# amathislab/BUCTD

Measured on AMD Instinct MI355X. Metric: images/sec (train) BUCTD-CoAM-W48 384x288, higher is better.
Workload: dtype f32 (3x3 convs: operands split exactly into 3 bf16 pieces, 6 bf16 MFMAs per product, fp32 accumulate - fp32-class); 1 GPU; BUCTD-CoAM-W48 (pose_hrnet_coam, ATT_MODULES [F,T,F,F], colored condition) 384x288 CrowdPose-14kpt full train step: fwd + JointsMSE + bwd + grad all-reduce + Adam + arg-max accuracy decode; global_batch=32, batch_per_gpu=32, input=N x 6 x 384 x 288 fp32, params=115581770, parallelism=dp1, hip_streams=4, conv_math=bf16x6, step_graph=False

## Files before the change

### buctd_amd/_C.py

```python
import ctypes as C
import os

import torch

_HERE = os.path.dirname(os.path.abspath(__file__))
LIB_PATH = os.path.join(_HERE, "lib", "libbuctd_hip.so")


class ConvDesc(C.Structure):
    _fields_ = [(n, C.c_int) for n in ("N", "H", "W", "Ci", "Co", "R", "S", "stride", "pad", "Ho", "Wo")]


class BasicBlockDesc(C.Structure):
    _fields_ = ([(n, C.c_int) for n in ("N", "H", "W", "C")] +
                [(n, C.c_void_p) for n in ("x", "w1_fwd", "w2_fwd", "w1_bwd", "w2_bwd", "gamma1", "beta1", "gamma2", "beta2",
                                           "running_mean1", "running_var1", "running_mean2", "running_var2")] +
                [(n, C.c_float) for n in ("eps1", "momentum1", "eps2", "momentum2")] +
                [(n, C.c_void_p) for n in ("z1", "z2", "y", "acc", "stat")])


class BasicBlockGrads(C.Structure):
    _fields_ = ([(n, C.c_void_p) for n in ("dy", "dz2", "dres", "dy1", "dz1", "dx", "dw1", "dw2", "dgamma1", "dbeta1",
                                           "dgamma2", "dbeta2")] +
                [(n, C.c_int) for n in ("acc_w1", "acc_w2", "acc_bn1", "acc_bn2")] +
                [("bn_acc", C.c_void_p), ("wg_ws", C.c_void_p), ("wg_ws_bytes", C.c_size_t)])


class BnAccIn(C.Structure):
    _fields_ = [("acc", C.c_void_p), ("rows", C.c_long), ("eps", C.c_float), ("momentum", C.c_float),
                ("mean_out", C.c_void_p), ("invstd_out", C.c_void_p), ("running_mean", C.c_void_p),
                ("running_var", C.c_void_p)]


class C3Conv(C.Structure):
    _fields_ = ([(n, C.c_int) for n in ("N", "H", "W", "Ci", "Co")] +
                [(n, C.c_void_p) for n in ("x", "wprep", "residual")] + [("relu", C.c_int)] +
                [(n, C.c_void_p) for n in ("y", "stats_acc")] + [("in_bn", C.POINTER(BnAccIn))] +
                [(n, C.c_void_p) for n in ("in_gamma", "in_beta")] + [("in_relu", C.c_int)] +
                [(n, C.c_void_p) for n in ("bn_z", "bn_y", "bn_mean", "bn_invstd", "bn_gamma", "bn_beta", "bn_acc")])


class C3ConvEval(C.Structure):
    _fields_ = ([(n, C.c_int) for n in ("N", "H", "W", "Ci", "Co")] +
                [(n, C.c_void_p) for n in ("x", "wprep", "scale", "shift", "residual")] + [("relu", C.c_int), ("y", C.c_void_p)])


class BnApplyItem(C.Structure):
    _fields_ = [("z", C.c_void_p), ("st", BnAccIn), ("gamma", C.c_void_p), ("beta", C.c_void_p), ("residual", C.c_void_p),
                ("relu", C.c_int), ("y", C.c_void_p), ("rows", C.c_long), ("C", C.c_int)]


class BnBwdItem(C.Structure):
    _fields_ = ([(n, C.c_void_p) for n in ("dy", "y", "z", "mean", "invstd", "gamma", "beta")] +
                [("relu", C.c_int), ("rows", C.c_long), ("C", C.c_int)] +
                [(n, C.c_void_p) for n in ("dz", "dres", "dgamma", "dbeta")] +
                [("accumulate", C.c_int), ("acc", C.c_void_p), ("acc_ready", C.c_int)])


class Wg3Conv(C.Structure):
    _fields_ = ([(n, C.c_int) for n in ("N", "H", "W", "Ci", "Co")] +
                [(n, C.c_void_p) for n in ("x", "dy", "dw")] + [("accumulate", C.c_int)] +
                [(n, C.c_void_p) for n in ("x_mean", "x_invstd", "x_gamma", "x_beta")] + [("x_relu", C.c_int)] +
                [("workspace", C.c_void_p), ("workspace_bytes", C.c_size_t)])


class MhaArgs(C.Structure):
    _fields_ = ([(n, C.c_int) for n in ("B", "T", "h", "dh")] +
                [(n, C.c_void_p) for n in ("q", "k", "v")] + [(n, C.c_int) for n in ("ldq", "ldk", "ldv")] +
                [("out", C.c_void_p), ("ldo", C.c_int), ("lse", C.c_void_p), ("scale", C.c_float), ("p_drop", C.c_float),
                 ("dout", C.c_void_p), ("lddo", C.c_int)] +
                [(n, C.c_void_p) for n in ("dq", "dk", "dv")] + [(n, C.c_int) for n in ("lddq", "lddk", "lddv")])


class AttnRowsArgs(C.Structure):
    _fields_ = ([(n, C.c_int) for n in ("B", "T", "h", "dh", "R")] + [("q", C.c_void_p), ("k", C.c_void_p)] +
                [("ldq", C.c_int), ("ldk", C.c_int), ("rows", C.c_void_p), ("scale", C.c_float), ("out", C.c_void_p),
                 ("out_heads", C.c_void_p)])


class RefineArgs(C.Structure):
    _fields_ = ([(n, C.c_void_p) for n in ("coords", "maxvals", "offset", "center", "scale", "box_score", "items",
                                           "cond_trunc", "cond_joints", "status", "hist_preds", "hist_score",
                                           "hist_box_score", "hist_keypoint_score", "hist_center", "hist_scale")] +
                [(n, C.c_int) for n in ("B", "K", "pass_", "passes", "heatmap_w", "heatmap_h", "crop_w", "crop_h")] +
                [(n, C.c_double) for n in ("margin", "aspect_ratio", "in_vis_thre", "scale_thre")])


class SampleGeomArgs(C.Structure):
    _fields_ = ([(n, C.c_void_p) for n in ("joints", "joints_vis", "cond", "cond_vis", "center", "scale", "bbox",
                                           "half_body", "draws", "bbox_draws", "flags", "pair", "items", "out_joints",
                                           "out_joints_vis", "out_cond", "out_cond_vis", "cond_trunc", "target_xy",
                                           "target_vis", "out_center", "out_scale", "out_rotation", "status")] +
                [(n, C.c_int) for n in ("B", "K", "crop_w", "crop_h", "keep_rect", "bbox_aug")] +
                [(n, C.c_double) for n in ("margin", "aspect_ratio", "scale_thre", "stride_x", "stride_y")])


class KptMatchArgs(C.Structure):
    _fields_ = ([(n, C.c_int) for n in ("images", "K", "n_thr", "n_area")] + [(n, C.c_long) for n in ("dt_total", "gt_total")] +
                [(n, C.c_void_p) for n in ("dt_offsets", "gt_offsets", "oks_offsets", "dt_kpts", "gt_kpts", "gt_area",
                                           "gt_bbox", "gt_flags", "sigmas", "thresholds", "area_ranges", "oks",
                                           "dt_matched", "dt_ignored")])


class VisCanvas(C.Structure):
    _fields_ = [("base", C.c_void_p), ("row_stride", C.c_long), ("H", C.c_int), ("W", C.c_int)]


class VisPoseArgs(C.Structure):
    _fields_ = ([(n, C.c_void_p) for n in ("canvases", "person_offsets", "persons", "joints", "skeleton", "palette",
                                           "tiles")] +
                [(n, C.c_int) for n in ("C", "P", "K", "L", "n_palette", "n_tiles", "canvas_h_max", "canvas_w_max",
                                        "style", "thickness", "radius")] +
                [("score_thresh", C.c_float), ("alpha256", C.c_int)])


VIS_POSE_PLAIN, VIS_POSE_PRETTY = 0, 1
VIS_POSE_TILE_W, VIS_POSE_TILE_H, VIS_POSE_CHUNK = 64, 16, 256


GRAD_SUMSQ_CHUNK = 8192

STEP_MAX_GROUPS, STEP_CHUNK = 16, 16384


class StepChunk(C.Structure):
    _fields_ = [("start", C.c_long), ("len", C.c_int), ("group", C.c_int)]


class AdamGroup(C.Structure):
    _fields_ = ([(n, C.c_float) for n in ("lr", "beta1", "beta2", "eps", "weight_decay")] +
                [("decoupled", C.c_int), ("step", C.c_int)])


class SgdGroup(C.Structure):
    _fields_ = [(n, C.c_float) for n in ("lr", "momentum", "weight_decay")] + [("nesterov", C.c_int)]


class AvgItem(C.Structure):
    _fields_ = [("src", C.c_void_p), ("avg", C.c_void_p), ("n", C.c_long)]


class MatmulDesc(C.Structure):
    _fields_ = [
        ("batch", C.c_int), ("M", C.c_int), ("N", C.c_int), ("K", C.c_int),
        ("a_layout", C.c_int), ("b_layout", C.c_int),
        ("lda", C.c_int), ("ldb", C.c_int), ("ldc", C.c_int),
        ("stride_a", C.c_long), ("stride_b", C.c_long), ("stride_c", C.c_long),
        ("Kc", C.c_int), ("group_stride_a", C.c_long), ("group_stride_bk", C.c_long),
        ("Nc", C.c_int), ("group_stride_bn", C.c_long), ("group_stride_c", C.c_long),
        ("alpha", C.c_float), ("bias_axis", C.c_int),
    ]


_P = C.c_void_p
_I = C.c_int
_L = C.c_long
_F = C.c_float
_D = C.c_double
_U64 = C.c_uint64
_SZ = C.c_size_t
_PD = C.POINTER(ConvDesc)
_PM = C.POINTER(MatmulDesc)
_PI = C.POINTER(C.c_int)
_PL = C.POINTER(C.c_long)

SIGNATURES = {
    "buctd_version": (_I, []),
    "buctd_last_error": (C.c_char_p, []),
    "buctd_conv2d_fwd": (_I, [_PD, _P, _P, _P, _P, _P, _P, _I, _P, _P, _P]),
    "buctd_conv2d_fwd_thin": (_I, [_PD]),
    "buctd_conv2d_dgrad": (_I, [_PD, _P, _P, _P, _P, _P, _P]),
    "buctd_conv2d_stats_groups": (_I, [_PD, _I, _PI, _PI]),
    "buctd_conv2d_wgrad_workspace": (_SZ, [_PD]),
    "buctd_conv2d_wgrad": (_I, [_PD, _P, _P, _P, _I, _P, _SZ, _P]),
    "buctd_conv2d_plan": (_I, [_PD, _I, _I, _PI]),
    "buctd_matmul_workspace": (_SZ, [_PM]),
    "buctd_matmul": (_I, [_PM, _P, _P, _P, _P, _P, _SZ, _P]),
    "buctd_matmul_plan": (_I, [_PM, _P, _P, _PI]),
    "buctd_bn_finalize": (_I, [_P, _P, _I, _I, _L, _I, _F, _F, _P, _P, _P, _P, _P]),
    "buctd_conv3x3_bf16x3_supported": (_I, [_I, _I, _I, _I, _I]),
    "buctd_conv3x3_bf16x3_stats_groups": (_I, [_I, _I, _I, _I, _I, _PI, _PI]),
    "buctd_conv3x3_bf16x3_prep_bytes": (_SZ, [_I, _I, _I]),
    "buctd_conv3x3_bf16x3_prep": (_I, [_I, _I, _P, _I, _P, _P]),
    "buctd_conv3x3_bf16x3_prep_batched": (_I, [_P, _I, _L, _P]),
    "buctd_conv3x3_bf16x3": (_I, [_I, _I, _I, _I, _I, _P, _P, _P, _P, _P, _P, _I, _P, _P, _P, _P]),
    "buctd_conv3x3_wgrad_bf16x3_supported": (_I, [_I, _I, _I, _I, _I]),
    "buctd_conv3x3_wgrad_bf16x3_workspace": (_SZ, [_I, _I, _I, _I, _I]),
    "buctd_conv3x3_wgrad_bf16x3": (_I, [_I, _I, _I, _I, _I, _P, _P, _P, _I, _P, _SZ, _P]),
    "buctd_conv3x3_bf16x6_supported": (_I, [_I, _I, _I, _I, _I]),
    "buctd_conv3x3_bf16x6_stats_groups": (_I, [_I, _I, _I, _I, _I, _PI, _PI]),
    "buctd_conv3x3_bf16x6_prep_bytes": (_SZ, [_I, _I, _I]),
    "buctd_conv3x3_bf16x6_prep": (_I, [_I, _I, _P, _I, _P, _P]),
    "buctd_conv3x3_bf16x6": (_I, [_I, _I, _I, _I, _I, _P, _P, _P, _P, _P, _P, _I, _P, _P, _P, _P]),
    "buctd_bn_bwd_from_partials": (_I, [_P, _P, _P, _P, _P, _P, _P, _I, _L, _I, _P, _I, _P, _P, _P, _P, _I, _P, _SZ, _P]),
    "buctd_conv3x3_wgrad_bf16x6_bnin": (_I, [_I, _I, _I, _I, _I, _P, _P, _P, _I, _P, _P, _P, _P, _I, _P, _SZ, _P]),
    "buctd_conv3x3_wgrad_bf16x6_supported": (_I, [_I, _I, _I, _I, _I]),
    "buctd_conv3x3_wgrad_bf16x6_workspace": (_SZ, [_I, _I, _I, _I, _I]),
    "buctd_conv3x3_wgrad_bf16x6": (_I, [_I, _I, _I, _I, _I, _P, _P, _P, _I, _P, _SZ, _P]),
    "buctd_bn_stats": (_I, [_P, _L, _I, _P, _PI, _PI, _P]),
    "buctd_bn_stats_groups": (_I, [_L, _I, _PI, _PI]),
    "buctd_bn_apply": (_I, [_P, _P, _P, _P, _P, _P, _I, _P, _L, _I, _P]),
    "buctd_bn_bwd_workspace": (_SZ, [_L, _I]),
    "buctd_bn_bwd": (_I, [_P, _P, _P, _P, _P, _P, _P, _I, _L, _I, _P, _P, _P, _P, _I, _P, _SZ, _P]),
    "buctd_bn_fold": (_I, [_P, _P, _P, _P, _F, _I, _P, _P, _P]),
    "buctd_bn_acc_bytes": (_SZ, [_I]),
    "buctd_bn_apply_acc": (_I, [_P, C.POINTER(BnAccIn), _P, _P, _P, _I, _P, _L, _I, _P]),
    "buctd_bn_bwd_acc": (_I, [_P, _P, _P, _P, _P, _P, _P, _I, _L, _I, _P, _P, _P, _P, _I, _P, _I, _P]),
    "buctd_conv3x3_bf16x6_acc": (_I, [_I] * 5 + [_P, _P, _P, _I, _P, _P, C.POINTER(BnAccIn), _P, _P, _I, _P]),
    "buctd_conv3x3_bf16x6_bnstat_acc": (_I, [_I] * 5 + [_P] * 12),
    "buctd_gconv_x6_fwd_acc": (_I, [_I] * 6 + [_P] * 6),
    "buctd_conv3x3_bf16x6_group": (_I, [_I, C.POINTER(C3Conv), _P]),
    "buctd_conv3x3_bf16x6_group_eval": (_I, [_I, C.POINTER(C3ConvEval), _P]),
    "buctd_conv3x3_bf16x6_group_workgroups": (_I, [_I, C.POINTER(C3Conv)]),
    "buctd_conv3x3_bf16x6_plan": (_I, [_I, _I, _I, _I, _I, _I, C.POINTER(C.c_int)]),
    "buctd_conv3x3_wgrad_bf16x6_plan": (_I, [_I, _I, _I, _I, _I, C.POINTER(C.c_int)]),
    "buctd_gconv_wgrad_x6_supported": (_I, [_I] * 6),
    "buctd_gconv_wgrad_x6_plan": (_I, [_I] * 6 + [C.POINTER(C.c_int)]),
    "buctd_gconv_wgrad_x6_workspace": (_SZ, [_I] * 6),
    "buctd_gconv_wgrad_x6": (_I, [_I] * 6 + [_P, _P, _P, _I, _P, _SZ, _P]),
    "buctd_bn_apply_acc_group": (_I, [_I, C.POINTER(BnApplyItem), _P]),
    "buctd_bn_bwd_acc_group": (_I, [_I, C.POINTER(BnBwdItem), _P]),
    "buctd_conv3x3_wgrad_bf16x6_group_workspace": (_SZ, [_I] * 6),
    "buctd_conv3x3_wgrad_bf16x6_group": (_I, [_I, C.POINTER(Wg3Conv), _P]),
    "buctd_conv3x3_wgrad_bf16x6_group_workgroups": (_I, [_I, C.POINTER(Wg3Conv)]),
    "buctd_stream_fork": (_I, [_P, _P]),
    "buctd_basic_branches_fwd_train": (_I, [_I, _I, C.POINTER(BasicBlockDesc), _P]),
    "buctd_basic_branches_bwd": (_I, [_I, _I, C.POINTER(BasicBlockDesc), C.POINTER(BasicBlockGrads), _P, _P]),
    "buctd_basic_chain_fwd_train": (_I, [_I, C.POINTER(BasicBlockDesc), _P]),
    "buctd_basic_chain_bwd": (_I, [_I, C.POINTER(BasicBlockDesc), C.POINTER(BasicBlockGrads), _P, _P]),
    "buctd_x6_image_dims": (_I, [_I, _I, _I, _P, _P]),
    "buctd_x6_image_bytes": (C.c_size_t, [_I, _I, _I]),
    "buctd_x6_image": (_I, [_P, _I, _I, _I, _L, _L, _I, _L, _L, _I, _P, _P]),
    "buctd_x6_gemm": (_I, [_I, _I, _I, _P, _P, _P, _I, _F, _P, _L, _I, _L, _P]),
    "buctd_x6_gemm_plan": (_I, [_I, _I, _I, _PI]),
    "buctd_x6_gemm_tile": (_I, [_I, _I, _I, _I, _PI, _PI]),
    "buctd_x6_image_path": (_I, [_P, _I, _I, _I, _L, _L, _I, _L, _L, _I, _I, _I, _PI]),
    "buctd_add": (_I, [_P, _P, _P, _L, _I, _P]),
    "buctd_add_n": (_I, [C.POINTER(_P), _I, _P, _L, _P]),
    "buctd_mul": (_I, [_P, _P, _P, _L, _P]),
    "buctd_scale": (_I, [_P, _P, _F, _P, _L, _P]),
    "buctd_copy_channels": (_I, [_P, _L, _I, _I, _P, _I, _I, _I, _P]),
    "buctd_add_bcast": (_I, [_P, _P, _P, _L, _L, _P]),
    "buctd_batch_sum": (_I, [_P, _L, _L, _P, _I, _P]),
    "buctd_relu_bwd": (_I, [_P, _P, _P, _L, _P]),
    "buctd_colsum_workspace": (_SZ, [_L, _I]),
    "buctd_colsum": (_I, [_P, _L, _I, _P, _I, _P, _SZ, _P]),
    "buctd_nchw_to_nhwc": (_I, [_P, _I, _I, _I, _I, _I, _I, _P, _P]),
    "buctd_nhwc_to_nchw": (_I, [_P, _I, _I, _I, _I, _P, _P]),
    "buctd_fuse_sum": (_I, [C.POINTER(_P), _PI, _I, _I, _I, _I, _I, _I, _P, _P]),
    "buctd_fuse_sum_bwd": (_I, [_P, _P, _I, _I, _I, _I, _I, _P, _P]),
    "buctd_resize_bilinear": (_I, [_P, _I, _I, _I, _I, _I, _I, _I, _I, _P, _P]),
    "buctd_maxpool3x3s2_fwd": (_I, [_P, _I, _I, _I, _I, _P, _P, _P]),
    "buctd_maxpool3x3s2_bwd": (_I, [_P, _P, _I, _I, _I, _I, _P, _P]),
    "buctd_softmax_dropout_fwd": (_I, [_P, _L, _I, _F, _F, _U64, _P, _P, _P]),
    "buctd_softmax_dropout_bwd": (_I, [_P, _P, _L, _I, _F, _F, _U64, _P, _P]),
    "buctd_softmax_dropout_fwd_dseed": (_I, [_P, _L, _I, _F, _F, _P, _P, _P, _P]),
    "buctd_softmax_dropout_bwd_dseed": (_I, [_P, _P, _L, _I, _F, _F, _P, _P, _P]),
    "buctd_dropout": (_I, [_P, _P, _L, _F, _U64, _P]),
    "buctd_dropout_dseed": (_I, [_P, _P, _L, _F, _P, _P]),
    "buctd_dropout_seed_fill": (_I, [_P, _I, _U64, _U64, _P]),
    "buctd_attn_smallqk_supported": (_I, [_I, _I, _I]),
    "buctd_attn_smallqk_plan": (_I, [_I, _I, _I, _I, _F, _I, _PI]),
    "buctd_attn_smallqk_fwd": (_I, [_I, _I, _I, _I, _P, _P, _P, _F, _F, _U64, _I, _P, _P, _P, _P]),
    "buctd_attn_smallqk_bwd": (_I, [_I, _I, _I, _I, _P, _P, _P, _P, _P, _P, _P, _F, _F, _U64, _I, _P, _P, _P, _P, _P]),
    "buctd_attn_smallqk_fwd_dseed": (_I, [_I, _I, _I, _I, _P, _P, _P, _F, _F, _P, _I, _P, _P, _P, _P]),
    "buctd_attn_smallqk_bwd_dseed": (_I, [_I, _I, _I, _I, _P, _P, _P, _P, _P, _P, _P, _F, _F, _P, _I, _P, _P, _P, _P, _P]),
    "buctd_layernorm_fwd": (_I, [_P, _P, _P, _L, _I, _F, _P, _P, _P, _P]),
    "buctd_add_layernorm_fwd": (_I, [_P, _P, _P, _P, _L, _I, _F, _P, _P, _P, _P, _P]),
    "buctd_layernorm_bwd_workspace": (_SZ, [_L, _I]),
    "buctd_layernorm_bwd": (_I, [_P, _P, _P, _P, _P, _L, _I, _P, _P, _P, _I, _P, _SZ, _P]),
    "buctd_joints_mse": (_I, [_P, _P, _P, _I, _I, _I, _P, _P, _F, _P, _SZ, _P]),
    "buctd_joints_ohkm_mse_workspace": (_SZ, [_I, _I]),
    "buctd_joints_ohkm_mse": (_I, [_P, _P, _P, _I, _I, _I, _I, _P, _P, _F, _P, _SZ, _P]),
    "buctd_argmax_decode": (_I, [_P, _I, _I, _I, _P, _P, _P, _P]),
    "buctd_warp_affine_norm": (_I, [_P, _I, _I, _I, _P, _P, _P, _L, _P, _P]),
    "buctd_cond_render_into": (_I, [_P, _I, _P, _I, _I, _I, _I, _I, _I, _P, _L, _P, _SZ, _P]),
    "buctd_cond_geometry": (_I, [_P, _P, _P, _P, _I, _I, _P, _P, _P, _P]),
    "buctd_cond_mirror": (_I, [_P, _I, _P, _P, _I, _I, _I, _P, _P]),
    "buctd_mirror_rows": (_I, [_P, _L, _P, _L, _P, _I, _I, _I, _I, _I, _P]),
    "buctd_refine_step": (_I, [C.POINTER(RefineArgs), _P]),
    "buctd_sample_geometry": (_I, [C.POINTER(SampleGeomArgs), _P]),
    "buctd_synthesize_pose": (_I, [_P, _P, _P, _P, _P, _P, _I, _I, _I, C.c_ulonglong, _P, _P]),
    "buctd_gconv_x6_supported": (_I, [_I] * 7),
    "buctd_gconv_x6_prep_bytes": (_SZ, [_I, _I, _I, _I]),
    "buctd_gconv_x6_prep": (_I, [_I, _I, _I, _P, _I, _P, _P]),
    "buctd_gconv_x6_prep_item_bytes": (_SZ, []),
    "buctd_gconv_x6_prep_item": (_I, [_I, _I, _I, _P, _I, _P, _P]),
    "buctd_gconv_x6_prep_batched": (_I, [_P, _I, _P]),
    "buctd_gconv_x6_stats_groups": (_I, [_I] * 6 + [_PI, _PI]),
    "buctd_gconv_x6_fwd": (_I, [_I] * 6 + [_P] * 6 + [_I, _P, _P, _P, _P]),
    "buctd_gconv_x6_dgrad": (_I, [_I] * 6 + [_P] * 4 + [_P]),
    "buctd_gconv_x6_plan": (_I, [_I] * 8 + [C.POINTER(C.c_int)]),
    "buctd_mha_fwd_bf16x6_workspace": (_SZ, [_I, _I, _I]),
    "buctd_mha_heads_fwd_bf16x6_ws": (_I, [C.POINTER(MhaArgs), _P, _SZ, _P]),
    "buctd_mha_heads_fwd_supported": (_I, [_I, _I, _I]),
    "buctd_mha_heads_fwd": (_I, [C.POINTER(MhaArgs), _P]),
    "buctd_mha_heads_fwd_bf16x6": (_I, [C.POINTER(MhaArgs), _P]),
    "buctd_mha_heads_train_supported": (_I, [_I, _I, _I]),
    "buctd_mha_heads_fwd_train": (_I, [C.POINTER(MhaArgs), _U64, _P]),
    "buctd_mha_heads_bwd_workspace": (_SZ, [_I, _I, _I]),
    "buctd_mha_heads_bwd": (_I, [C.POINTER(MhaArgs), _U64, _P, _SZ, _P]),
    "buctd_mha_heads_fwd_train_dseed": (_I, [C.POINTER(MhaArgs), _P, _P]),
    "buctd_mha_heads_bwd_dseed": (_I, [C.POINTER(MhaArgs), _P, _P, _SZ, _P]),
    "buctd_attn_rows_supported": (_I, [_I, _I, _I]),
    "buctd_attn_rows": (_I, [C.POINTER(AttnRowsArgs), _P]),
    "buctd_nms_workspace": (_SZ, [_I]),
    "buctd_nms": (_I, [_P, _P, _P, _I, _I, _F, _P, _SZ, _P]),
    "buctd_cpu_nms": (_I, [_P, _I, _P, _F, _P, _P]),
    "buctd_kpt_rescore": (_I, [_P, _P, _I, _I, _D, _P, _P, _P, _P]),
    "buctd_oks_nms_grouped": (_I, [_P, _I, _I, _P, _P, _P, _I, _D, _I, _D, _P, _P]),
    "buctd_coco_kpt_match_workspace": (_SZ, [_L, _I, _I]),
    "buctd_coco_kpt_match": (_I, [C.POINTER(KptMatchArgs), _P, _SZ, _P]),
    "buctd_kpt_crowding": (_I, [_P, _I, _L, _I, _P, _P, _P, _P, _D, _P, _P, _P]),
    "buctd_kpt_segment_ap": (_I, [_P, _I, _I, _L, _P, _P, _I, _I, _P, _P, _I, _I, _I, _P, _P, _P]),
    "buctd_pose_boxes": (_I, [_P, _I, _I, _I, _P, _D, _P, _P, _P]),
    "buctd_match_boxes": (_I, [_P, _P, _I, _P, _P, _P, _P, _P, _P]),
    "buctd_group_max_iou": (_I, [_P, _I, _P, _I, _P, _P, _P, _P]),
    "buctd_group_near_list": (_I, [_P, _I, _P, _P, _P, _P]),
    "buctd_vis_minmax": (_I, [_P, _I, _I, _I, _L, _L, _L, _L, _P, _P]),
    "buctd_vis_heatmap_grid": (_I, [_P, _I, _I, _I, _L, _L, _L, _L, _P, _P, _I, _I, _I, _P, _I, _P, _P]),
    "buctd_vis_joint_grid": (_I, [_P, _I, _I, _I, _L, _L, _L, _L, _P, _I, _P, _P, _P, _P, _P, _P, _I, _I, _I, _P, _P]),
    "buctd_vis_pose_overlay": (_I, [C.POINTER(VisPoseArgs), _P]),
    "buctd_argmax_decode_refined": (_I, [_P, _I, _I, _I, _P, _P, _P, _P, _P]),
    "buctd_argmax_decode_dark": (_I, [_P, _I, _I, _I, _P, _P, _P, _P, _P]),
    "buctd_gaussian_target": (_I, [_P, _P, _I, _I, _I, _I, _F, _F, _F, _P, _P, _P]),
    "buctd_cond_render_workspace": (_SZ, [_I, _I, _I, _I]),
    "buctd_cond_render": (_I, [_P, _I, _P, _I, _I, _I, _I, _I, _I, _P, _P, _SZ, _P]),
    "buctd_flipback_avg": (_I, [_P, _P, _P, _I, _I, _I, _I, _I, _P, _P]),
    "buctd_sgd_step": (_I, [_P, _P, _P, _L, _F, _F, _F, _I, _I, _F, _P]),
    "buctd_adam_step": (_I, [_P, _P, _P, _P, _L, _F, _F, _F, _F, _I, _F, _P]),
    "buctd_sgd_step_dscale": (_I, [_P, _P, _P, _L, _F, _F, _F, _I, _I, _F, _P, _P]),
    "buctd_adam_step_dscale": (_I, [_P, _P, _P, _P, _L, _F, _F, _F, _F, _I, _F, _P, _P]),
    "buctd_step_chunks": (_L, [_PL, _PI, _I, C.POINTER(StepChunk)]),
    "buctd_adam_step_groups": (_I, [_P, _P, _P, _P, _P, _L, C.POINTER(AdamGroup), _I, _F, _P, _P]),
    "buctd_sgd_step_groups": (_I, [_P, _P, _P, _P, _L, C.POINTER(SgdGroup), _I, _F, _P, _P]),
    "buctd_grad_sumsq_workspace": (_SZ, [_PL, _I]),
    "buctd_grad_sumsq": (_I, [_P, _PL, _I, _P, _P, _SZ, _P]),
    "buctd_grad_clip_coef": (_I, [_P, _D, _D, _P, _P, _P]),
    "buctd_grad_segment_stats": (_I, [_P, _P, _I, _P, _P, _P]),
    "buctd_ema_update": (_I, [_P, _P, _L, _F, _P]),
    "buctd_ema_update_tensors": (_I, [_P, _I, _F, _P]),
    "buctd_swap": (_I, [_P, _P, _L, _P]),
    "buctd_bf16_pack_conv": (_I, [_P, _L, _L, _L, _L, _I, _I, _I, _P, _P, _P, _P, _P, _F, _P, _P, _P]),
    "buctd_bf16_conv": (_I, [_P, _I, _I, _I, _I, _P, _P, _I, _I, _I, _I, _P, _I, _I, _P, _P, _SZ, _P]),
    "buctd_bf16_fuse_sum": (_I, [C.POINTER(_P), _PI, _I, _I, _I, _I, _I, _I, _P, _P]),
    "buctd_bf16_from_f32": (_I, [_P, _L, _P, _P]),
}

_lib = None


class BuctdHipError(RuntimeError):
    pass


def lib():
    global _lib
    if _lib is None:
        if not os.path.isfile(LIB_PATH):
            raise BuctdHipError(
                f"{LIB_PATH} is missing - build it with `make` (or __graft_entry__.build()); "
                "buctd_amd has no CPU / eager fallback")
        handle = C.CDLL(LIB_PATH, mode=C.RTLD_GLOBAL)
        for name, (res, args) in SIGNATURES.items():
            fn = getattr(handle, name)
            fn.restype = res
            fn.argtypes = args
        _lib = handle
    return _lib


def check(rc, what=""):
    if rc != 0:
        msg = lib().buctd_last_error()
        raise BuctdHipError(f"{what} failed ({rc}): {msg.decode() if msg else ''}")


_raw_stream = getattr(torch._C, "_cuda_getCurrentRawStream", None)
_raw_device = getattr(torch._C, "_cuda_getDevice", None)


def current_stream_handle():
# ... 16 lines not shown
```

### buctd_amd/csrc/block.hip

```cpp
#include "common.h"
#include "../../include/buctd_hip.h"
#include <string.h>

#define BLK_TRY(call)      \
  do {                     \
    const int rc_ = (call); \
    if (rc_) return rc_;   \
  } while (0)

static bool fwd_ptrs_ok(const buctd_basic_block& b) {
  return b.x && b.w1_fwd && b.w2_fwd && b.z1 && b.z2 && b.y && b.acc && b.stat;
}

static bool bwd_ptrs_ok(const buctd_basic_block& b, const buctd_basic_block_grads& g) {
  return b.x && b.w1_bwd && b.w2_bwd && b.z1 && b.z2 && b.y && b.stat && g.dy && g.dres && g.dy1 && g.dw1 && g.dw2 && g.bn_acc &&
         g.wg_ws && g.dz2 && g.dz1;
}


static float* mean1_of(const buctd_basic_block& b) { return b.stat; }
static float* invstd1_of(const buctd_basic_block& b) { return b.stat + b.C; }
static float* mean2_of(const buctd_basic_block& b) { return b.stat + 2 * b.C; }
static float* invstd2_of(const buctd_basic_block& b) { return b.stat + 3 * b.C; }
static void* acc1_of(void* acc) { return acc; }
static void* acc2_of(void* acc, int C) { return (char*)acc + buctd_bn_acc_bytes(C); }

static void acc_in_of(const buctd_basic_block& b, int second, buctd_bn_acc_in* st) {
  st->acc = second ? acc2_of(b.acc, b.C) : acc1_of(b.acc);
  st->rows = (long)b.N * b.H * b.W;
  st->eps = second ? b.eps2 : b.eps1;
  st->momentum = second ? b.momentum2 : b.momentum1;
  st->mean_out = second ? mean2_of(b) : mean1_of(b);
  st->invstd_out = second ? invstd2_of(b) : invstd1_of(b);
  st->running_mean = second ? b.running_mean2 : b.running_mean1;
  st->running_var = second ? b.running_var2 : b.running_var1;
}

static buctd_c3_conv c3_of(const buctd_basic_block& b) {
  buctd_c3_conv c;
  memset(&c, 0, sizeof(c));
  c.N = b.N; c.H = b.H; c.W = b.W; c.Ci = c.Co = b.C;
  return c;
}

static int stream_fork(hipStream_t from, hipStream_t to, const char* who) {
  if (from == to) return BUCTD_OK;
  static thread_local hipEvent_t evs[16] = {nullptr};
  int devid = 0;
  if (hipGetDevice(&devid) != hipSuccess || devid < 0 || devid >= 16) {
    buctd_set_error("%s: cannot identify the current device", who);
    return BUCTD_ELAUNCH;
  }
  hipEvent_t& ev = evs[devid];
  if (!ev && hipEventCreateWithFlags(&ev, hipEventDisableTiming) != hipSuccess) {
    buctd_set_error("%s: hipEventCreate failed", who);
    return BUCTD_ELAUNCH;
  }
  if (hipEventRecord(ev, from) != hipSuccess || hipStreamWaitEvent(to, ev, 0) != hipSuccess) {
    buctd_set_error("%s: stream fork failed", who);
    return BUCTD_ELAUNCH;
  }
  return BUCTD_OK;
}

static int issue_conv_fwd(bool group, int n, const buctd_c3_conv* c, void* s) {
  if (group) return buctd_conv3x3_bf16x6_group(n, c, s);
  return buctd_conv3x3_bf16x6_acc(c->N, c->H, c->W, c->Ci, c->Co, c->x, c->wprep, c->residual, c->relu, c->y, c->stats_acc,
                                  c->in_bn, c->in_gamma, c->in_beta, c->in_relu, s);
}
static int issue_dgrad(bool group, int n, const buctd_c3_conv* c, void* s) {
  if (group) return buctd_conv3x3_bf16x6_group(n, c, s);
  if (c->bn_acc)
    return buctd_conv3x3_bf16x6_bnstat_acc(c->N, c->H, c->W, c->Ci, c->Co, c->x, c->wprep, c->residual, c->y, c->bn_z, c->bn_y,
                                           c->bn_mean, c->bn_invstd, c->bn_gamma, c->bn_beta, c->bn_acc, s);
  return buctd_conv3x3_bf16x6(c->N, c->H, c->W, c->Ci, c->Co, c->x, c->wprep, nullptr, nullptr, nullptr, c->residual, 0, c->y,
                              nullptr, nullptr, s);
}
static int issue_wgrad(bool group, int n, const buctd_wg3_conv* c, void* s) {
  if (group) return buctd_conv3x3_wgrad_bf16x6_group(n, c, s);
  if (c->x_mean)
    return buctd_conv3x3_wgrad_bf16x6_bnin(c->N, c->H, c->W, c->Ci, c->Co, c->x, c->dy, c->dw, c->accumulate, c->x_mean,
                                           c->x_invstd, c->x_gamma, c->x_beta, c->x_relu, c->workspace, c->workspace_bytes, s);
  return buctd_conv3x3_wgrad_bf16x6(c->N, c->H, c->W, c->Ci, c->Co, c->x, c->dy, c->dw, c->accumulate, c->workspace,
                                    c->workspace_bytes, s);
}
static int issue_bn_apply(bool group, int n, const buctd_bn_apply_item* a, void* s) {
  if (group) return buctd_bn_apply_acc_group(n, a, s);
  return buctd_bn_apply_acc(a->z, &a->st, a->gamma, a->beta, a->residual, a->relu, a->y, a->rows, a->C, s);
}
static int issue_bn_bwd(bool group, int n, const buctd_bn_bwd_item* i, void* s) {
  if (group) return buctd_bn_bwd_acc_group(n, i, s);
  return buctd_bn_bwd_acc(i->dy, i->y, i->z, i->mean, i->invstd, i->gamma, i->beta, i->relu, i->rows, i->C, i->dz, i->dres,
                          i->dgamma, i->dbeta, i->accumulate, i->acc, i->acc_ready, s);
}

#define BR_MAX 4

static int row_fwd_train(bool group, int nb, int n, const buctd_basic_block* blocks, void* stream) {
  for (int k = 0; k < n; ++k) {
    buctd_c3_conv cv[BR_MAX];
    buctd_bn_acc_in st1[BR_MAX];
    buctd_bn_apply_item ap[BR_MAX];
    for (int b = 0; b < nb; ++b) {
      const buctd_basic_block& B = blocks[b * n + k];
      buctd_c3_conv& c = cv[b] = c3_of(B);
      c.x = B.x; c.wprep = B.w1_fwd; c.y = B.z1; c.stats_acc = acc1_of(B.acc);
    }
    BLK_TRY(issue_conv_fwd(group, nb, cv, stream));
    for (int b = 0; b < nb; ++b) {
      const buctd_basic_block& B = blocks[b * n + k];
      buctd_c3_conv& c = cv[b];
      acc_in_of(B, 0, &st1[b]);
      c.x = B.z1; c.wprep = B.w2_fwd; c.y = B.z2; c.stats_acc = acc2_of(B.acc, B.C);
      c.in_bn = &st1[b]; c.in_gamma = B.gamma1; c.in_beta = B.beta1; c.in_relu = 1;
    }
    BLK_TRY(issue_conv_fwd(group, nb, cv, stream));
    for (int b = 0; b < nb; ++b) {
      const buctd_basic_block& B = blocks[b * n + k];
      buctd_bn_apply_item& a = ap[b];
      a.z = B.z2;
      acc_in_of(B, 1, &a.st);
      a.gamma = B.gamma2; a.beta = B.beta2; a.residual = B.x; a.relu = 1; a.y = B.y;
      a.rows = a.st.rows; a.C = B.C;
    }
    BLK_TRY(issue_bn_apply(group, nb, ap, stream));
  }
  return BUCTD_OK;
}

static bool bn2_sums_chain(const buctd_basic_block* b, const buctd_basic_block_grads* g) {
  return g->dx && g->dx == g[-1].dy && g[-1].bn_acc && b[-1].y == b->x && b[-1].N == b->N && b[-1].H == b->H && b[-1].W == b->W &&
         b[-1].C == b->C;
}

static int row_bwd(bool group, const char* who, int nb, int n, const buctd_basic_block* blocks,
                   const buctd_basic_block_grads* grads, void* stream, void* side_stream) {
  hipStream_t main_s = (hipStream_t)stream, side_s = side_stream ? (hipStream_t)side_stream : main_s;
  bool ready[BR_MAX] = {false, false, false, false};
  for (int k = n - 1; k >= 0; --k) {
    buctd_bn_bwd_item bi[BR_MAX];
    buctd_wg3_conv wg[BR_MAX];
    buctd_c3_conv cv[BR_MAX];
    bool chain[BR_MAX];
    for (int b = 0; b < nb; ++b) {
      const buctd_basic_block& B = blocks[b * n + k];
      const buctd_basic_block_grads& G = grads[b * n + k];
      chain[b] = k > 0 && bn2_sums_chain(&B, &G);
      bi[b] = buctd_bn_bwd_item{G.dy, B.y, B.z2, mean2_of(B), invstd2_of(B), B.gamma2, nullptr, 1, (long)B.N * B.H * B.W, B.C,
                                G.dz2, G.dres, G.dgamma2, G.dbeta2, G.acc_bn2, acc2_of(G.bn_acc, B.C), ready[b] ? 1 : 0};
    }
    BLK_TRY(issue_bn_bwd(group, nb, bi, stream));
    BLK_TRY(stream_fork(main_s, side_s, who));
    for (int b = 0; b < nb; ++b) {
      const buctd_basic_block& B = blocks[b * n + k];
      const buctd_basic_block_grads& G = grads[b * n + k];
      wg[b] = buctd_wg3_conv{B.N, B.H, B.W, B.C, B.C, B.z1, G.dz2, G.dw2, G.acc_w2, mean1_of(B), invstd1_of(B), B.gamma1, B.beta1,
                             1, G.wg_ws, G.wg_ws_bytes};
    }
    BLK_TRY(issue_wgrad(group, nb, wg, side_s));
    for (int b = 0; b < nb; ++b) {
      const buctd_basic_block& B = blocks[b * n + k];
      const buctd_basic_block_grads& G = grads[b * n + k];
      buctd_c3_conv& c = cv[b] = c3_of(B);
      c.x = G.dz2; c.wprep = B.w2_bwd; c.y = G.dy1;
      c.bn_z = B.z1; c.bn_mean = mean1_of(B); c.bn_invstd = invstd1_of(B); c.bn_gamma = B.gamma1; c.bn_beta = B.beta1;
      c.bn_acc = acc1_of(G.bn_acc);
    }
    BLK_TRY(issue_dgrad(group, nb, cv, stream));
    for (int b = 0; b < nb; ++b) {
      const buctd_basic_block& B = blocks[b * n + k];
      const buctd_basic_block_grads& G = grads[b * n + k];
      bi[b] = buctd_bn_bwd_item{G.dy1, nullptr, B.z1, mean1_of(B), invstd1_of(B), B.gamma1, B.beta1, 1, (long)B.N * B.H * B.W, B.C,
                                G.dz1, nullptr, G.dgamma1, G.dbeta1, G.acc_bn1, acc1_of(G.bn_acc), 1};
    }
    BLK_TRY(issue_bn_bwd(group, nb, bi, stream));
    BLK_TRY(stream_fork(main_s, side_s, who));
    for (int b = 0; b < nb; ++b) {
      const buctd_basic_block& B = blocks[b * n + k];
      const buctd_basic_block_grads& G = grads[b * n + k];
      wg[b] = buctd_wg3_conv{B.N, B.H, B.W, B.C, B.C, B.x, G.dz1, G.dw1, G.acc_w1, nullptr, nullptr, nullptr, nullptr, 0,
                             G.wg_ws, G.wg_ws_bytes};
    }
    BLK_TRY(issue_wgrad(group, nb, wg, side_s));
    int m = 0;
    for (int b = 0; b < nb; ++b) {
      const buctd_basic_block& B = blocks[b * n + k];
      const buctd_basic_block_grads& G = grads[b * n + k];
      ready[b] = chain[b];
      if (!G.dx) continue;
      buctd_c3_conv& c = cv[m++] = c3_of(B);
      c.x = G.dz1; c.wprep = B.w1_bwd; c.residual = G.dres; c.y = G.dx;
      if (chain[b]) {
        const buctd_basic_block& Bp = blocks[b * n + k - 1];
        c.bn_z = Bp.z2; c.bn_y = Bp.y; c.bn_mean = mean2_of(Bp); c.bn_invstd = invstd2_of(Bp); c.bn_gamma = Bp.gamma2;
        c.bn_acc = acc2_of(grads[b * n + k - 1].bn_acc, B.C);
      }
    }
    if (m) BLK_TRY(issue_dgrad(group, m, cv, stream));
  }
  return BUCTD_OK;
}

extern "C" int buctd_basic_chain_fwd_train(int n, const buctd_basic_block* blocks, void* stream) {
  BUCTD_CHECK_ARG(n > 0 && blocks, "buctd_basic_chain_fwd_train: bad argument");
  for (int k = 0; k < n; ++k) BUCTD_CHECK_ARG(fwd_ptrs_ok(blocks[k]), "buctd_basic_chain_fwd_train: null pointer in block %d", k);
  return row_fwd_train(false, 1, n, blocks, stream);
}
extern "C" int buctd_basic_chain_bwd(int n, const buctd_basic_block* blocks, const buctd_basic_block_grads* grads, void* stream,
                                     void* side_stream) {
  BUCTD_CHECK_ARG(n > 0 && blocks && grads, "buctd_basic_chain_bwd: bad argument");
  for (int k = 0; k < n; ++k)
    BUCTD_CHECK_ARG(bwd_ptrs_ok(blocks[k], grads[k]), "buctd_basic_chain_bwd: null pointer in block %d", k);
  return row_bwd(false, "buctd_basic_chain_bwd", 1, n, blocks, grads, stream, side_stream);
}

extern "C" int buctd_basic_branches_fwd_train(int nb, int n, const buctd_basic_block* blocks, void* stream) {
  BUCTD_CHECK_ARG(nb > 0 && nb <= BR_MAX && n > 0 && blocks, "buctd_basic_branches_fwd_train: 1..%d branches", BR_MAX);
  for (int i = 0; i < nb * n; ++i)
    BUCTD_CHECK_ARG(fwd_ptrs_ok(blocks[i]), "buctd_basic_branches_fwd_train: null pointer in block %d", i);
  return row_fwd_train(true, nb, n, blocks, stream);
}
extern "C" int buctd_basic_branches_bwd(int nb, int n, const buctd_basic_block* blocks, const buctd_basic_block_grads* grads,
                                        void* stream, void* side_stream) {
  BUCTD_CHECK_ARG(nb > 0 && nb <= BR_MAX && n > 0 && blocks && grads, "buctd_basic_branches_bwd: 1..%d branches", BR_MAX);
  for (int i = 0; i < nb * n; ++i)
    BUCTD_CHECK_ARG(bwd_ptrs_ok(blocks[i], grads[i]), "buctd_basic_branches_bwd: null pointer in block %d", i);
  return row_bwd(true, "buctd_basic_branches_bwd", nb, n, blocks, grads, stream, side_stream);
}

extern "C" int buctd_stream_fork(void* from, void* to) {
  return stream_fork((hipStream_t)from, (hipStream_t)to, "buctd_stream_fork");
}
```

### buctd_amd/csrc/bn.hip

```cpp
#include "common.h"
#include "../../include/buctd_hip.h"
#include "bn_acc.h"

#define STAT_ROWS 64

__global__ __launch_bounds__(256) void bn_stats_kernel(const float* __restrict__ z, long rows, int C,
                                                       float* __restrict__ part) {
  const long r0 = (long)blockIdx.x * STAT_ROWS;
  long r1 = r0 + STAT_ROWS;
  if (r1 > rows) r1 = rows;
  const int cnt = (int)(r1 - r0);
  for (int c = threadIdx.x; c < C; c += 256) {
    float s = 0.f;
    for (long r = r0; r < r1; ++r) s += z[r * C + c];
    const float mean = cnt > 0 ? s / (float)cnt : 0.f;
    float m2 = 0.f;
    for (long r = r0; r < r1; ++r) {
      const float d = z[r * C + c] - mean;
      m2 += d * d;
    }
    part[((long)blockIdx.x * C + c) * 2 + 0] = mean;
    part[((long)blockIdx.x * C + c) * 2 + 1] = m2;
  }
}
// ... 760 lines not shown
      f32x4 g[4], zz[4], yy[4];
#pragma unroll
      for (int u = 0; u < 4; ++u) {
        const long o = (r + u * step) * c4n + tc;
        g[u] = reinterpret_cast<const f32x4*>(dy)[o];
        zz[u] = reinterpret_cast<const f32x4*>(z)[o];
        yy[u] = (relu && y) ? reinterpret_cast<const f32x4*>(y)[o] : zz[u];
      }
#pragma unroll
      for (int u = 0; u < 4; ++u) body(g[u], zz[u], yy[u]);
    }
    for (; r < r1; r += step) {
      const long o = r * c4n + tc;
      const f32x4 zz = reinterpret_cast<const f32x4*>(z)[o];
      body(reinterpret_cast<const f32x4*>(dy)[o], zz, (relu && y) ? reinterpret_cast<const f32x4*>(y)[o] : zz);
    }
  }
  sm[0][threadIdx.x] = s1;
  sm[1][threadIdx.x] = s2;
  __syncthreads();
  if (tr == 0) {
    for (int k = 1; k < rl; ++k) {
      s1 += sm[0][k * c4n + tc];
      s2 += sm[1][k * c4n + tc];
    }
    sm[0][tc] = s1;
    sm[1][tc] = s2;
  }
  __syncthreads();
  const unsigned shard = bnacc_shard();
  for (int c = threadIdx.x; c < C; c += 256)
    bnacc_add(acc, C, shard, c, (double)reinterpret_cast<const float*>(&sm[0][0])[c], (double)reinterpret_cast<const float*>(&sm[1][0])[c]);
}
__global__ __launch_bounds__(256) void bn_bwd_reduce_acc_kernel(BnBwdArgs p) {
  __shared__ f32x4 sm[2][256];
  bn_bwd_reduce_acc_body(p, blockIdx.x, sm);
}
__global__ __launch_bounds__(256) void bn_bwd_reduce_acc_group_kernel(BnGroup<BnBwdArgs> g_) {
  __shared__ f32x4 sm[2][256];
  const BnGroup<BnBwdArgs>& g = *(const BnGroup<BnBwdArgs>*)__builtin_amdgcn_kernarg_segment_ptr();
  unsigned bid, nblk;
  const int k = bn_group_find(g, &bid, &nblk);
  bn_bwd_reduce_acc_body(g.s[k], bid, sm);
}

__device__ __forceinline__ void bn_bwd_apply_acc_body(const BnBwdArgs& p, unsigned bid, unsigned nblk, unsigned char* lds_raw) {
  const float* __restrict__ dy = p.dy;
  const float* __restrict__ y = p.y;
  const float* __restrict__ z = p.z;
  const float* __restrict__ mean = p.mean;
  const float* __restrict__ invstd = p.invstd;
  const float* __restrict__ gamma = p.gamma;
  const float* __restrict__ beta = p.beta;
  const long long* __restrict__ acc = p.acc;
  float* __restrict__ dz = p.dz;
  float* __restrict__ dres = p.dres;
  float* __restrict__ dgamma = p.dgamma;
  float* __restrict__ dbeta = p.dbeta;
  const int relu = p.relu, C = p.C, accumulate = p.accumulate;
  const long total = p.rows * C;
  const float inv_rows = p.inv_rows;
  long long* wsum = reinterpret_cast<long long*>(lds_raw);
  float* tab = reinterpret_cast<float*>(lds_raw + (size_t)BNACC_WORDS * C * sizeof(long long));
  const long n4 = total >> 2;
  const long step = (long)nblk * 256;
  const bool ld_y = relu && y;
  long i = (long)bid * 256 + threadIdx.x;
  f32x4 g0 = (f32x4){0.f, 0.f, 0.f, 0.f}, g1 = g0, z0 = g0, z1 = g0, y0 = g0, y1 = g0;
  auto fetch = [&](long j) {
    if (j < n4) {
      g0 = reinterpret_cast<const f32x4*>(dy)[j];
      z0 = reinterpret_cast<const f32x4*>(z)[j];
      if (ld_y) y0 = reinterpret_cast<const f32x4*>(y)[j];
    }
    if (j + step < n4) {
      g1 = reinterpret_cast<const f32x4*>(dy)[j + step];
      z1 = reinterpret_cast<const f32x4*>(z)[j + step];
      if (ld_y) y1 = reinterpret_cast<const f32x4*>(y)[j + step];
    }
  };
  fetch(i);
  bnacc_gather_lds(acc, C, wsum);
  for (int c = threadIdx.x; c < C; c += 256) {
    double s1, s2;
    bnacc_read_lds(wsum, C, c, &s1, &s2);
    tab[c] = mean[c];
    tab[C + c] = invstd[c];
    tab[2 * C + c] = gamma[c];
    tab[3 * C + c] = (relu && !y) ? beta[c] : 0.f;
    tab[4 * C + c] = (float)s1;
    tab[5 * C + c] = (float)s2;
    if (bid == 0) {
      if (dbeta) dbeta[c] = accumulate ? dbeta[c] + (float)s1 : (float)s1;
      if (dgamma) dgamma[c] = accumulate ? dgamma[c] + (float)s2 : (float)s2;
    }
  }
  __syncthreads();
  const int dc = (int)((step * 4) % C);
  int c = (int)((i * 4) % C) - dc;
  auto one = [&](long j, int cc, f32x4 g, f32x4 zz, f32x4 yy) {
    const f32x4 mu = *reinterpret_cast<const f32x4*>(tab + cc);
    const f32x4 is = *reinterpret_cast<const f32x4*>(tab + C + cc);
    const f32x4 ga = *reinterpret_cast<const f32x4*>(tab + 2 * C + cc);
    if (relu) {
      if (!y) {
        const f32x4 be = *reinterpret_cast<const f32x4*>(tab + 3 * C + cc);
#pragma unroll
        for (int j4 = 0; j4 < 4; ++j4) {
          const float sc = is[j4] * ga[j4];
          yy[j4] = (zz[j4] - mu[j4]) * sc + be[j4];
        }
      }
#pragma unroll
      for (int j4 = 0; j4 < 4; ++j4)
        if (!(yy[j4] > 0.f)) g[j4] = 0.f;
    }
    const f32x4 s1 = *reinterpret_cast<const f32x4*>(tab + 4 * C + cc);
    const f32x4 s2 = *reinterpret_cast<const f32x4*>(tab + 5 * C + cc);
    f32x4 o;
#pragma unroll
    for (int j4 = 0; j4 < 4; ++j4) {
      const float zh = (zz[j4] - mu[j4]) * is[j4];
      o[j4] = ga[j4] * is[j4] * (g[j4] - s1[j4] * inv_rows - zh * s2[j4] * inv_rows);
    }
    reinterpret_cast<f32x4*>(dz)[j] = o;
    if (dres) reinterpret_cast<f32x4*>(dres)[j] = g;
  };
  for (; i < n4; i += 2 * step) {
    c += dc;
    if (c >= C) c -= C;
    one(i, c, g0, z0, y0);
    c += dc;
    if (c >= C) c -= C;
    if (i + step < n4) one(i + step, c, g1, z1, y1);
    fetch(i + 2 * step);
  }
}
__global__ __launch_bounds__(256, 6) void bn_bwd_apply_acc_kernel(BnBwdArgs p) {
  extern __shared__ __attribute__((aligned(16))) unsigned char lds_raw[];
  bn_bwd_apply_acc_body(p, blockIdx.x, gridDim.x, lds_raw);
}
__global__ __launch_bounds__(256, 6) void bn_bwd_apply_acc_group_kernel(BnGroup<BnBwdArgs> g_) {
  extern __shared__ __attribute__((aligned(16))) unsigned char lds_raw[];
  const BnGroup<BnBwdArgs>& g = *(const BnGroup<BnBwdArgs>*)__builtin_amdgcn_kernarg_segment_ptr();
  unsigned bid, nblk;
  const int k = bn_group_find(g, &bid, &nblk);
  bn_bwd_apply_acc_body(g.s[k], bid, nblk, lds_raw);
}

static int bn_bwd_acc_fill(const buctd_bn_bwd_item& it, const char* who, BnBwdArgs& a, long* nb) {
  BUCTD_CHECK_ARG(it.dy && it.z && it.mean && it.invstd && it.gamma && it.dz && it.acc && it.rows > 0 && it.C > 0 && it.C % 4 == 0 &&
                      it.C / 4 <= 256,
                  "%s: bad argument (C must be a multiple of 4, <= 1024)", who);
  BUCTD_CHECK_ARG(!it.relu || it.y || it.beta, "%s: relu backward needs the forward output, or beta to rebuild its sign", who);
  a.dy = it.dy; a.y = it.y; a.z = it.z; a.mean = it.mean; a.invstd = it.invstd; a.gamma = it.gamma; a.beta = it.beta;
  a.acc = (long long*)it.acc; a.relu = it.relu; a.rows = it.rows; a.C = it.C;
  *nb = bwd2_blocks(it.rows, &a.rows_per_block);
  a.inv_rows = 1.0f / (float)it.rows;
  a.dz = it.dz; a.dres = it.dres; a.dgamma = it.dgamma; a.dbeta = it.dbeta; a.accumulate = it.accumulate;
  return BUCTD_OK;
}

extern "C" int buctd_bn_bwd_acc(const float* dy, const float* y, const float* z, const float* mean, const float* invstd,
                                const float* gamma, const float* beta, int relu, long rows, int C, float* dz, float* dres,
                                float* dgamma, float* dbeta, int accumulate, void* acc, int acc_ready, void* stream) {
  const buctd_bn_bwd_item it{dy, y, z, mean, invstd, gamma, beta, relu, rows, C, dz, dres, dgamma, dbeta, accumulate, acc, acc_ready};
  BnBwdArgs a;
  long nb;
  const int rc = bn_bwd_acc_fill(it, "buctd_bn_bwd_acc", a, &nb);
  if (rc) return rc;
  hipStream_t st = (hipStream_t)stream;
  if (!acc_ready) {
    hipLaunchKernelGGL(bn_bwd_reduce_acc_kernel, dim3((unsigned)nb), dim3(256), 0, st, a);
    BUCTD_CHECK_LAUNCH("buctd_bn_bwd_acc(reduce)");
  }
  const long total = rows * C;
  hipLaunchKernelGGL(bn_bwd_apply_acc_kernel, dim3(acc_grid(total / 4, 6)), dim3(256), (size_t)(BNACC_WORDS * 8 + 6 * 4) * C, st, a);
  BUCTD_CHECK_LAUNCH("buctd_bn_bwd_acc(apply)");
  return BUCTD_OK;
}

extern "C" int buctd_bn_bwd_acc_group(int n, const buctd_bn_bwd_item* items, void* stream) {
  BUCTD_CHECK_ARG(n > 0 && n <= BNG_MAX && items, "buctd_bn_bwd_acc_group: 1..%d tensors", BNG_MAX);
  BnGroup<BnBwdArgs> ga, gr;
  ga.n = n; gr.n = 0;
  ga.first[0] = gr.first[0] = 0;
  size_t lds = 0;
  for (int k = 0; k < n; ++k) {
    long nb;
    const int rc = bn_bwd_acc_fill(items[k], "buctd_bn_bwd_acc_group", ga.s[k], &nb);
    if (rc) return rc;
    const long total = items[k].rows * items[k].C;
    ga.first[k + 1] = ga.first[k] + (unsigned)acc_grid(total / 4, 6);
    const size_t l = (size_t)(BNACC_WORDS * 8 + 6 * 4) * items[k].C;
    if (l > lds) lds = l;
    if (!items[k].acc_ready) {
      gr.s[gr.n] = ga.s[k];
      gr.first[gr.n + 1] = gr.first[gr.n] + (unsigned)nb;
      ++gr.n;
    }
  }
  for (int k = n; k < BNG_MAX; ++k) ga.first[k + 1] = ga.first[n];
  for (int k = gr.n; k < BNG_MAX; ++k) gr.first[k + 1] = gr.first[gr.n];
  hipStream_t st = (hipStream_t)stream;
  if (gr.n) {
    hipLaunchKernelGGL(bn_bwd_reduce_acc_group_kernel, dim3(gr.first[gr.n]), dim3(256), 0, st, gr);
    BUCTD_CHECK_LAUNCH("buctd_bn_bwd_acc_group(reduce)");
  }
  hipLaunchKernelGGL(bn_bwd_apply_acc_group_kernel, dim3(ga.first[n]), dim3(256), lds, st, ga);
  BUCTD_CHECK_LAUNCH("buctd_bn_bwd_acc_group(apply)");
  return BUCTD_OK;
}
```

### buctd_amd/csrc/c3_common.h

```cpp
#pragma once
#include "common.h"
#include <stdlib.h>
#include "../../include/buctd_hip.h"
#include "bn_acc.h"

typedef __bf16 bf16x8 __attribute__((ext_vector_type(8)));
typedef unsigned short u16x4 __attribute__((ext_vector_type(4)));

#define CK 32

template <int NP> struct Geo;
template <> struct Geo<2> {
  static constexpr int ROWB = 160;
  static constexpr int PST = 64;
  static constexpr int CPR = 8;
  static constexpr int BROW = 128;
  static constexpr int BLDS = 160;
};
template <> struct Geo<3> {
  static constexpr int ROWB = 96;
  static constexpr int PST = 32;
  static constexpr int CPR = 4;
  static constexpr int BROW = 192;
  static constexpr int BLDS = 224;
};

struct C3Args {
  const float* x;
  const unsigned char* wp;
  float* out;
  const float* bias;
  const float* scale;
  const float* shift;
  const float* res;
  float* stats;
  int* counts;
  int N, H, W, Ci, Co;
  int SW, IB, P;
  int relu, na;
  const float* in_gamma;
  const float* in_beta;
  int in_relu;
  int col_major;
  unsigned ib_mul, ib_sh, sw_mul, sw_sh;
  int omap, oH, oW, ost, oy0, ox0;
  const float* bs_z;
  const float* bs_y;
  const float* bs_mean;
  const float* bs_invstd;
  const float* bs_gamma;
  const float* bs_beta;
  long long* stats_acc;
  long long* bs_acc;
  BnAccFwd in_acc;
};

#define C3G_MAX 4
struct C3Group {
  C3Args conv[C3G_MAX];
  int nconv;
  int tiles[C3G_MAX];
  int gx[C3G_MAX];
  int gy[C3G_MAX];
  int variant[C3G_MAX];
};

#define C3_EPI_EXCH_OFF 24576
#define C3_EPI_LDS (C3_EPI_EXCH_OFF + 256 * 16)

__device__ __forceinline__ int fast_div(int n, unsigned mul, unsigned sh) {
  return (int)(__umulhi((unsigned)n, mul) >> sh);
}

typedef float c3_f32x2 __attribute__((ext_vector_type(2)));
typedef __bf16 c3_bf16x2 __attribute__((ext_vector_type(2)));
typedef unsigned c3_u32x2 __attribute__((ext_vector_type(2)));
template <int NP, int PST>
__device__ __forceinline__ void split_store_pk(unsigned char* row, int c, f32x4 v) {
  c3_f32x2 lo = {v.x, v.y}, hi = {v.z, v.w};
#pragma unroll
  for (int q = 0; q < NP; ++q) {
    const unsigned a = __builtin_bit_cast(unsigned, __builtin_convertvector(lo, c3_bf16x2));
    const unsigned b = __builtin_bit_cast(unsigned, __builtin_convertvector(hi, c3_bf16x2));
    *reinterpret_cast<c3_u32x2*>(row + q * PST + 2 * c) = (c3_u32x2){a, b};
    if (q + 1 < NP) {
      lo -= (c3_f32x2){__uint_as_float(a << 16), __uint_as_float(a & 0xffff0000u)};
      hi -= (c3_f32x2){__uint_as_float(b << 16), __uint_as_float(b & 0xffff0000u)};
    }
  }
}

template <int NP, int PST>
__device__ __forceinline__ void split_store(unsigned char* row, int c, f32x4 v) {
#pragma unroll
  for (int q = 0; q < NP; ++q) {
    u16x4 pc;
#pragma unroll
    for (int j = 0; j < 4; ++j) {
      const __bf16 h = (__bf16)v[j];
      pc[j] = __builtin_bit_cast(unsigned short, h);
      v[j] -= (float)h;
    }
    *reinterpret_cast<u16x4*>(row + q * PST + 2 * c) = pc;
  }
}

#define MAX_SW 75

static inline int c3_row_width(int W) { return W + 1; }

template <int V>
struct IC { static constexpr int value = V; };

template <int MF, int NF, int WM, int WN>
__device__ __forceinline__ void c3_epilogue(const C3Args& p, f32x4 (&acc)[MF][NF], unsigned char* smem, int bx, int by,
                                            int p0, int n0) {
  const int t = threadIdx.x, lane = t & 63, wave = t >> 6;
  const int i16 = lane & 15, g = lane >> 4;
  const int wave_m = wave % WM, wave_n = wave / WM;
  constexpr int MR = MF * 16;
  constexpr int RH = (MR + 63) / 64;
  constexpr int LD = NF * 16 + 4;
  constexpr int EP = 1;
  static_assert(MR <= 128, "c3_epilogue: at most 128 rows per wave");
  float* stg = reinterpret_cast<float*>(smem) + wave * (EP * 16 * LD);
  int* rowoff = reinterpret_cast<int*>(smem) + 4 * EP * 16 * LD + wave * 128;
  unsigned long long vmask[RH];
  int cnt = 0;
#pragma unroll
  for (int h = 0; h < RH; ++h) {
    int myoff = -1;
    const int r = lane + 64 * h;
    if (r < MR) {
      const int pp = p0 + wave_m * MR + r;
      if (pp < p.P) {
        const int n = fast_div(pp, p.ib_mul, p.ib_sh);
        const int rem = pp - n * p.IB;
        const int yy = fast_div(rem, p.sw_mul, p.sw_sh), xx = rem - yy * p.SW;
        if (n < p.N && yy >= 1 && xx >= 1 && xx <= p.W)
          myoff = p.omap ? ((n * p.oH + (yy - 1) * p.ost + p.oy0) * p.oW + (xx - 1) * p.ost + p.ox0) * p.Co
                         : ((n * p.H + yy - 1) * p.W + xx - 1) * p.Co;
      }
    }
    vmask[h] = __ballot(myoff >= 0);
    cnt += __popcll(vmask[h]);
    rowoff[r] = myoff;
  }
  auto valid = [&](int row) -> bool { return (vmask[row >> 6] >> (row & 63)) & 1ull; };
  const int grp = bx * WM + wave_m;
  if (p.stats && p.counts && by == 0 && wave_n == 0 && lane == 0) p.counts[grp] = cnt;
  const int ncol0 = n0 + wave_n * NF * 16;
  float bv[NF];
#pragma unroll
  for (int nf = 0; nf < NF; ++nf) bv[nf] = p.bias ? p.bias[ncol0 + nf * 16 + i16] : 0.f;
  double2* exch = reinterpret_cast<double2*>(smem + C3_EPI_EXCH_OFF);
  if (p.stats || p.stats_acc) {
    const float inv_cnt = cnt > 0 ? 1.f / (float)cnt : 0.f;
#pragma unroll
    for (int nf = 0; nf < NF; ++nf) {
      float s1 = 0.f;
#pragma unroll
      for (int mf = 0; mf < MF; ++mf)
#pragma unroll
        for (int rg = 0; rg < 4; ++rg) s1 += valid(mf * 16 + g * 4 + rg) ? acc[mf][nf][rg] + bv[nf] : 0.f;
      s1 += __shfl_xor(s1, 16, 64);
      s1 += __shfl_xor(s1, 32, 64);
      const float mean = s1 * inv_cnt;
      float s2 = 0.f;
#pragma unroll
      for (int mf = 0; mf < MF; ++mf)
#pragma unroll
        for (int rg = 0; rg < 4; ++rg) {
          const float d = acc[mf][nf][rg] + bv[nf] - mean;
          s2 += valid(mf * 16 + g * 4 + rg) ? d * d : 0.f;
        }
      s2 += __shfl_xor(s2, 16, 64);
      s2 += __shfl_xor(s2, 32, 64);
      if (g == 0) {
        const int n = ncol0 + nf * 16 + i16;
        if (p.stats) *reinterpret_cast<float2*>(p.stats + ((long)grp * p.Co + n) * 2) = make_float2(mean, s2);
        if (p.stats_acc) {
          const double nn = (double)cnt, m = (double)mean;
          exch[wave_m * (WN * NF * 16) + wave_n * NF * 16 + nf * 16 + i16] = make_double2(nn * m, (double)s2 + nn * m * m);
        }
      }
    }
    if (p.stats_acc) {
      __syncthreads();
      if (t < WN * NF * 16) {
        double a1 = 0.0, a2 = 0.0;
#pragma unroll
        for (int w = 0; w < WM; ++w) {
          const double2 v = exch[w * (WN * NF * 16) + t];
          a1 += v.x;
          a2 += v.y;
        }
        bnacc_add(p.stats_acc, p.Co, bnacc_shard(), n0 + t, a1, a2);
      }
    }
  }
  constexpr int Q4 = NF * 4;
  constexpr int NACC = (64 % Q4 == 0) ? 1 : 3;
  static_assert(NF <= 4 && (64 % Q4 == 0 || Q4 == 12), "c3_epilogue: unexpected column count for the bs reduction");
  f32x4 bs1[NACC], bs2[NACC];
#pragma unroll
  for (int j = 0; j < NACC; ++j) bs1[j] = bs2[j] = (f32x4){0.f, 0.f, 0.f, 0.f};
  const bool bs_on = p.bs_acc != nullptr;
  const bool bs_rebuild = bs_on && p.bs_y == nullptr;
#define C3_EPI_SYNC() __builtin_amdgcn_wave_barrier()
  constexpr int NI = EP * NF;
  constexpr int NPASS = MF / EP;
  f32x4 pre_r[2][NI], pre_z[2][NI], pre_y[2][NI];
  const bool has_res = p.res != nullptr;
  const bool has_y = bs_on && !bs_rebuild;
  C3_EPI_SYNC();
  auto issue = [&](int ps, int buf) {
#pragma unroll
    for (int k = 0; k < NI; ++k) {
      const int item = lane + 64 * k;
      const int row = item / (NF * 4), c4 = item - row * (NF * 4);
      const int off = rowoff[ps * EP * 16 + row];
      const int o = off >= 0 ? off + ncol0 + c4 * 4 : 0;
      if (has_res) pre_r[buf][k] = *reinterpret_cast<const f32x4*>(p.res + o);
      if (bs_on) pre_z[buf][k] = *reinterpret_cast<const f32x4*>(p.bs_z + o);
      if (has_y) pre_y[buf][k] = *reinterpret_cast<const f32x4*>(p.bs_y + o);
    }
  };
  if (has_res || bs_on) issue(0, 0);
#pragma unroll
  for (int ps = 0; ps < NPASS; ++ps) {
    if (ps) C3_EPI_SYNC();
    if ((has_res || bs_on) && ps + 1 < NPASS) issue(ps + 1, (ps + 1) & 1);
#pragma unroll
    for (int e = 0; e < EP; ++e)
#pragma unroll
      for (int nf = 0; nf < NF; ++nf)
#pragma unroll
        for (int rg = 0; rg < 4; ++rg)
          stg[(e * 16 + g * 4 + rg) * LD + nf * 16 + i16] = acc[ps * EP + e][nf][rg] + bv[nf];
    C3_EPI_SYNC();
#pragma unroll
    for (int k = 0; k < NI; ++k) {
      const int item = lane + 64 * k;
      const int row = item / (NF * 4), c4 = item - row * (NF * 4);
      f32x4 v = *reinterpret_cast<const f32x4*>(stg + row * LD + c4 * 4);
      const int off = rowoff[ps * EP * 16 + row];
      const int n = ncol0 + c4 * 4;
      if (off >= 0) {
        if (p.scale) {
          const f32x4 sc = *reinterpret_cast<const f32x4*>(p.scale + n);
          const f32x4 sh = *reinterpret_cast<const f32x4*>(p.shift + n);
#pragma unroll
          for (int j = 0; j < 4; ++j) v[j] = v[j] * sc[j] + sh[j];
        }
        if (has_res) {
          const f32x4 r = pre_r[ps & 1][k];
#pragma unroll
          for (int j = 0; j < 4; ++j) v[j] += r[j];
        }
        if (p.relu) {
#pragma unroll
          for (int j = 0; j < 4; ++j) v[j] = fmaxf(v[j], 0.f);
        }
        *reinterpret_cast<f32x4*>(p.out + off + n) = v;
        if (bs_on) {
          const f32x4 zz = pre_z[ps & 1][k];
          const f32x4 mu = *reinterpret_cast<const f32x4*>(p.bs_mean + n);
          const f32x4 is = *reinterpret_cast<const f32x4*>(p.bs_invstd + n);
          f32x4 yy;
          if (bs_rebuild) {
            const f32x4 sc = is * *reinterpret_cast<const f32x4*>(p.bs_gamma + n);
            yy = (zz - mu) * sc + *reinterpret_cast<const f32x4*>(p.bs_beta + n);
          } else {
            yy = pre_y[ps & 1][k];
          }
          f32x4 gm = v;
#pragma unroll
          for (int j = 0; j < 4; ++j)
            if (!(yy[j] > 0.f)) gm[j] = 0.f;
          bs1[k % NACC] += gm;
          bs2[k % NACC] += gm * (zz - mu) * is;
        }
      }
    }
  }
  if (bs_on) {
    __syncthreads();
    f32x4* red = reinterpret_cast<f32x4*>(smem) + (size_t)wave * (NACC * 64 * 2);
#pragma unroll
    for (int j = 0; j < NACC; ++j) {
      red[(j * 64 + lane) * 2 + 0] = bs1[j];
      red[(j * 64 + lane) * 2 + 1] = bs2[j];
    }
    __syncthreads();
    if (lane < Q4) {
      f32x4 a1 = (f32x4){0.f, 0.f, 0.f, 0.f}, a2 = a1;
#pragma unroll
      for (int j = 0; j < NACC; ++j) {
        const int first = ((lane - (64 * j) % Q4) % Q4 + Q4) % Q4;
        for (int l = first; l < 64; l += Q4) {
          a1 += red[(j * 64 + l) * 2 + 0];
          a2 += red[(j * 64 + l) * 2 + 1];
        }
      }
#pragma unroll
      for (int j = 0; j < 4; ++j)
        exch[wave_m * (WN * NF * 16) + wave_n * NF * 16 + lane * 4 + j] = make_double2((double)a1[j], (double)a2[j]);
    }
    __syncthreads();
    if (t < WN * NF * 16) {
      double a1 = 0.0, a2 = 0.0;
#pragma unroll
      for (int w = 0; w < WM; ++w) {
        const double2 v = exch[w * (WN * NF * 16) + t];
        a1 += v.x;
        a2 += v.y;
      }
      bnacc_add(p.bs_acc, p.Co, bnacc_shard(), n0 + t, a1, a2);
    }
  }
}


static inline void magic_u32(unsigned d, unsigned* mul, unsigned* sh) {
  if (d == 1) { *mul = 0xFFFFFFFFu; *sh = 0; return; }
  unsigned l = 0;
  while ((1ull << l) < d) ++l;
  const unsigned long long m = ((1ull << (31 + l)) + d - 1) / d;
  *mul = (unsigned)m;
  *sh = l - 1;
}
```

### buctd_amd/csrc/c3_lean.h

```cpp
#pragma once
#include "c3_common.h"

enum { C3M_IN_BN = 1, C3M_STATS = 2, C3M_RES = 4, C3M_BS_REBUILD = 8, C3M_BS_Y = 16 };

#define C3_OOB 0x80000000u
__device__ __forceinline__ __amdgpu_buffer_rsrc_t c3_rsrc(const void* ptr, unsigned bytes) {
  return __builtin_amdgcn_make_buffer_rsrc(const_cast<void*>(ptr), 0, bytes, 0x00020000);
}
__device__ __forceinline__ f32x4 c3_bload(__amdgpu_buffer_rsrc_t r, unsigned off) {
  typedef unsigned u32x4_ __attribute__((ext_vector_type(4)));
  return __builtin_bit_cast(f32x4, __builtin_amdgcn_raw_buffer_load_b128(r, off, 0, 0));
}
__device__ __forceinline__ void c3_bstore(__amdgpu_buffer_rsrc_t r, unsigned off, f32x4 v) {
  typedef unsigned u32x4_ __attribute__((ext_vector_type(4)));
  __builtin_amdgcn_raw_buffer_store_b128(__builtin_bit_cast(u32x4_, v), r, off, 0, 0);
}

static inline size_t c3l_tab_bytes(int Ci, int BN) { return (size_t)3 * Ci * 4 + (size_t)4 * BN * 4; }

template <int MF, int NF, int WM, int WN, int MODE>
__device__ __forceinline__ void c3l_epilogue(const C3Args& p, f32x4 (&acc)[MF][NF], unsigned char* smem, float* tab, int p0,
                                             int n0) {
  constexpr bool STATS = (MODE & C3M_STATS) != 0, RES = (MODE & C3M_RES) != 0;
  constexpr bool BSR = (MODE & C3M_BS_REBUILD) != 0, BSY = (MODE & C3M_BS_Y) != 0, BS = BSR || BSY;
  static_assert(!(STATS && BS), "c3l_epilogue: forward statistics and backward sums never meet in one launch");
  const int t = threadIdx.x, lane = t & 63;
  const int wave = __builtin_amdgcn_readfirstlane(t >> 6);
  const int i16 = lane & 15, g = lane >> 4;
  const int wave_m = wave % WM, wave_n = wave / WM;
  constexpr int MR = MF * 16;
  constexpr int RH = (MR + 63) / 64;
  constexpr int LD = NF * 16 + 4;
  constexpr int BN = WN * NF * 16;
  constexpr int Q4 = NF * 4;
  constexpr int NACC = (64 % Q4 == 0) ? 1 : 3;
  constexpr int NI = NF;
  static_assert(MR <= 128 && NF <= 4 && (64 % Q4 == 0 || Q4 == 12), "c3l_epilogue: unexpected tile shape");
  float* stg = reinterpret_cast<float*>(smem) + wave * (16 * LD);
  int* rowoff = reinterpret_cast<int*>(smem) + 4 * 16 * LD + wave * 128;
  double2* exch = reinterpret_cast<double2*>(smem + C3_EPI_EXCH_OFF);

  const int oH = p.omap ? p.oH : p.H, oW = p.omap ? p.oW : p.W, ost = p.omap ? p.ost : 1;
  const int oy0 = p.omap ? p.oy0 : 0, ox0 = p.omap ? p.ox0 : 0;
  const unsigned obytes = (unsigned)p.N * oH * oW * p.Co * 4u;
  const __amdgpu_buffer_rsrc_t r_out = c3_rsrc(p.out, obytes);
  int cnt = 0;
  int r0 = -1;
#pragma unroll
  for (int h = 0; h < RH; ++h) {
    unsigned myoff = C3_OOB;
    const int r = lane + 64 * h;
    const int pp = p0 + wave_m * MR + r;
    const int n = fast_div(pp, p.ib_mul, p.ib_sh);
    const int rem = pp - n * p.IB;
    const int yy = fast_div(rem, p.sw_mul, p.sw_sh), xx = rem - yy * p.SW;
    if ((r < MR) & (pp < p.P) & (n < p.N) & (yy >= 1) & (xx >= 1) & (xx <= p.W))
      myoff = (unsigned)(((n * oH + (yy - 1) * ost + oy0) * oW + (xx - 1) * ost + ox0) * p.Co) * 4u;
    if (STATS) {
      const unsigned long long vm = __ballot(myoff != C3_OOB);
      cnt += __popcll(vm);
      if (r0 < 0 && vm) r0 = 64 * h + __builtin_ctzll(vm);
    }
    if (r < MR) reinterpret_cast<unsigned*>(rowoff)[r] = myoff;
  }
  const int ncol0 = n0 + wave_n * NF * 16;
  float* piv = tab + wave * (NF * 16);
  const float* btab = tab + wave_n * NF * 16;
  if constexpr (STATS) {
    r0 = r0 < 0 ? 0 : r0;
    const int mf0 = r0 >> 4, g0 = (r0 >> 2) & 3, rg0 = r0 & 3;
    float pv[NF];
#pragma unroll
    for (int nf = 0; nf < NF; ++nf) pv[nf] = 0.f;
#pragma unroll
    for (int mf = 0; mf < MF; ++mf)
      if (mf == mf0) {
#pragma unroll
        for (int nf = 0; nf < NF; ++nf)
          pv[nf] = rg0 == 0 ? acc[mf][nf][0] : rg0 == 1 ? acc[mf][nf][1] : rg0 == 2 ? acc[mf][nf][2] : acc[mf][nf][3];
      }
    if (g == g0) {
#pragma unroll
      for (int nf = 0; nf < NF; ++nf) piv[nf * 16 + i16] = pv[nf];
    }
  }
  __builtin_amdgcn_wave_barrier();

  const float* sp[NI];
  const unsigned* rp[NI];
  int c4_k[NI];
#pragma unroll
  for (int k = 0; k < NI; ++k) {
    const int item = lane + 64 * k;
    const int row = item / Q4;
    c4_k[k] = item - row * Q4;
    sp[k] = stg + row * LD + c4_k[k] * 4;
    rp[k] = reinterpret_cast<const unsigned*>(rowoff) + row;
  }
  const unsigned colb = (unsigned)ncol0 * 4u;
  f32x4 s1[NACC], s2[NACC], pq[NACC];
#pragma unroll
  for (int j = 0; j < NACC; ++j) {
    s1[j] = s2[j] = (f32x4){0.f, 0.f, 0.f, 0.f};
    if constexpr (STATS) pq[j] = *reinterpret_cast<const f32x4*>(piv + c4_k[j] * 4);
  }
  [[maybe_unused]] __amdgpu_buffer_rsrc_t r_res, r_z, r_y;
  if constexpr (RES) r_res = c3_rsrc(p.res, obytes);
  if constexpr (BS) r_z = c3_rsrc(p.bs_z, obytes);
  if constexpr (BSY) r_y = c3_rsrc(p.bs_y, obytes);
  f32x4 pre_r[2][RES ? NI : 1], pre_z[2][BS ? NI : 1], pre_y[2][BSY ? NI : 1];
  auto issue = [&](int ps, int buf) {
#pragma unroll
    for (int k = 0; k < NI; ++k) {
      const unsigned o = rp[k][ps * 16] + colb + c4_k[k] * 16;
      if constexpr (RES) pre_r[buf][k] = c3_bload(r_res, o);
      if constexpr (BS) pre_z[buf][k] = c3_bload(r_z, o);
      if constexpr (BSY) pre_y[buf][k] = c3_bload(r_y, o);
    }
  };
  if constexpr (RES || BS) issue(0, 0);
#pragma unroll
  for (int ps = 0; ps < MF; ++ps) {
    if (ps) __builtin_amdgcn_wave_barrier();
    if constexpr (RES || BS) {
      if (ps + 1 < MF) issue(ps + 1, (ps + 1) & 1);
    }
#pragma unroll
    for (int nf = 0; nf < NF; ++nf)
#pragma unroll
      for (int rg = 0; rg < 4; ++rg) stg[(g * 4 + rg) * LD + nf * 16 + i16] = acc[ps][nf][rg];
    __builtin_amdgcn_wave_barrier();
    f32x4 v[NI];
    unsigned off[NI];
#pragma unroll
    for (int k = 0; k < NI; ++k) {
      v[k] = *reinterpret_cast<const f32x4*>(sp[k]);
      off[k] = rp[k][ps * 16];
    }
#pragma unroll
    for (int k = 0; k < NI; ++k) {
      const bool ok = off[k] != C3_OOB;
      if constexpr (RES) v[k] += pre_r[ps & 1][k];
      c3_bstore(r_out, off[k] + colb + c4_k[k] * 16, v[k]);
      if constexpr (STATS) {
        f32x4 d = v[k] - pq[k % NACC];
#pragma unroll
        for (int j = 0; j < 4; ++j) d[j] = ok ? d[j] : 0.f;
        s1[k % NACC] += d;
        f32x4 q = s2[k % NACC];
#pragma unroll
        for (int j = 0; j < 4; ++j) q[j] = __builtin_fmaf(d[j], d[j], q[j]);
        s2[k % NACC] = q;
      }
      if constexpr (BS) {
        const f32x4 zz = pre_z[ps & 1][k];
        const f32x4 mu = *reinterpret_cast<const f32x4*>(btab + c4_k[k] * 4);
        const f32x4 is = *reinterpret_cast<const f32x4*>(btab + BN + c4_k[k] * 4);
        f32x4 yy;
        if constexpr (BSR) {
          const f32x4 sc = *reinterpret_cast<const f32x4*>(btab + 2 * BN + c4_k[k] * 4);
          yy = (zz - mu) * sc + *reinterpret_cast<const f32x4*>(btab + 3 * BN + c4_k[k] * 4);
        } else {
          yy = pre_y[ps & 1][k];
        }
        f32x4 gm;
#pragma unroll
        for (int j = 0; j < 4; ++j) gm[j] = (ok && yy[j] > 0.f) ? v[k][j] : 0.f;
        s1[k % NACC] += gm;
        f32x4 tm = gm * (zz - mu) * is;
        s2[k % NACC] += tm;
      }
    }
    if constexpr (STATS || BS) {
#pragma unroll
      for (int j = 0; j < NACC; ++j) asm volatile("" : "+v"(s1[j]), "+v"(s2[j]));
    }
  }
  if constexpr (STATS || BS) {
    __syncthreads();
    f32x4* red = reinterpret_cast<f32x4*>(smem) + (size_t)wave * (NACC * 64 * 2);
#pragma unroll
    for (int j = 0; j < NACC; ++j) {
      red[(j * 64 + lane) * 2 + 0] = s1[j];
      red[(j * 64 + lane) * 2 + 1] = s2[j];
    }
    __builtin_amdgcn_wave_barrier();
    if (lane < Q4) {
      if constexpr (BS) {
        f32x4 a1 = (f32x4){0.f, 0.f, 0.f, 0.f}, a2 = a1;
#pragma unroll
        for (int j = 0; j < NACC; ++j) {
          const int first = ((lane - (64 * j) % Q4) % Q4 + Q4) % Q4;
          for (int l = first; l < 64; l += Q4) {
            a1 += red[(j * 64 + l) * 2 + 0];
            a2 += red[(j * 64 + l) * 2 + 1];
          }
        }
#pragma unroll
        for (int j = 0; j < 4; ++j)
          exch[wave_m * BN + wave_n * NF * 16 + lane * 4 + j] = make_double2((double)a1[j], (double)a2[j]);
      } else {
        double a1[4] = {0.0, 0.0, 0.0, 0.0}, a2[4] = {0.0, 0.0, 0.0, 0.0};
#pragma unroll
        for (int j = 0; j < NACC; ++j) {
          const int first = ((lane - (64 * j) % Q4) % Q4 + Q4) % Q4;
          for (int l = first; l < 64; l += Q4) {
            const f32x4 u1 = red[(j * 64 + l) * 2 + 0], u2 = red[(j * 64 + l) * 2 + 1];
#pragma unroll
            for (int e = 0; e < 4; ++e) {
              a1[e] += (double)u1[e];
              a2[e] += (double)u2[e];
            }
          }
        }
        const double nn = (double)cnt;
#pragma unroll
        for (int e = 0; e < 4; ++e) {
          const double pi = (double)piv[lane * 4 + e];
          exch[wave_m * BN + wave_n * NF * 16 + lane * 4 + e] =
              make_double2(a1[e] + nn * pi, a2[e] + 2.0 * pi * a1[e] + nn * pi * pi);
        }
      }
    }
    __syncthreads();
    if (t < BN) {
      double a1 = 0.0, a2 = 0.0;
#pragma unroll
      for (int w = 0; w < WM; ++w) {
        const double2 v = exch[w * BN + t];
        a1 += v.x;
        a2 += v.y;
      }
      bnacc_add(STATS ? p.stats_acc : p.bs_acc, p.Co, bnacc_shard(), n0 + t, a1, a2);
    }
  }
}

template <int BM, bool IN_BN>
struct C3Stager {
  static constexpr int ROWB = Geo<3>::ROWB, PST = Geo<3>::PST, CPR = Geo<3>::CPR;
  static constexpr int RPP = 256 / CPR;
  static constexpr int PA = (BM + 2 * MAX_SW + 2 + RPP - 1) / RPP;
  static constexpr int P0 = (BM + 2 * 3 + 2) / RPP < PA ? (BM + 2 * 3 + 2) / RPP : PA;
  unsigned goff[PA], lrow[PA];
  f32x4 areg[PA];
  int arows, c4, prow;
  __amdgpu_buffer_rsrc_t r_x;

  __device__ __forceinline__ void init(const C3Args& p) {
    const int t = threadIdx.x;
    arows = p.na * 32;
    c4 = (t % CPR) * 4;
    prow = t / CPR;
    r_x = c3_rsrc(p.x, (unsigned)p.N * p.H * p.W * p.Ci * 4u);
#pragma unroll
    for (int q = 0; q < PA; ++q) {
      const int row = prow + RPP * q;
      lrow[q] = (unsigned)(row < arows ? row : arows - 1) * ROWB + 2 * c4;
    }
  }
  __device__ __forceinline__ void make(const C3Args& p, int p0) {
    const int halo = p.SW + 1;
#pragma unroll
    for (int q = 0; q < PA; ++q) {
      const int row = prow + RPP * q;
      const int pp = p0 - halo + row;
      const int n = fast_div(pp, p.ib_mul, p.ib_sh);
      const int rem = pp - n * p.IB;
      const int yy = fast_div(rem, p.sw_mul, p.sw_sh);
      const int xx = rem - yy * p.SW;
      const bool real = (row < arows) & (pp >= 0) & (pp < p.P) & (n < p.N) & (yy >= 1) & (xx >= 1) & (xx <= p.W);
      goff[q] = real ? (unsigned)(((n * p.H + yy - 1) * p.W + xx - 1) * p.Ci + c4) * 4u : C3_OOB;
    }
  }
  __device__ __forceinline__ void load(int c0) {
#pragma unroll
    for (int q = 0; q < P0; ++q) areg[q] = c3_bload(r_x, goff[q] + (unsigned)c0 * 4u);
#pragma unroll
    for (int q0 = P0; q0 < PA; q0 += 2)
      if (RPP * q0 < arows) {
        areg[q0] = c3_bload(r_x, goff[q0] + (unsigned)c0 * 4u);
        if (q0 + 1 < PA) areg[q0 + 1] = c3_bload(r_x, goff[q0 + 1] + (unsigned)c0 * 4u);
      }
  }
  __device__ __forceinline__ void store_pass(const C3Args& p, unsigned char* At, int q, const f32x4& mu, const f32x4& sc,
                                             const f32x4& be) {
    f32x4 v = areg[q];
    if constexpr (IN_BN) {
      const bool real = goff[q] != C3_OOB;
#pragma unroll
      for (int j = 0; j < 4; ++j) {
        const float u = (v[j] - mu[j]) * sc[j] + be[j];
        const float w = p.in_relu ? fmaxf(u, 0.f) : u;
        v[j] = real ? w : 0.f;
      }
// ... 183 lines not shown
```

### buctd_amd/csrc/conv3x3.hip

```cpp
#include "c3_common.h"
#include <string.h>

enum { C3M_IN_BN = 1, C3M_STATS = 2, C3M_RES = 4, C3M_BS_REBUILD = 8, C3M_BS_Y = 16 };
int c3_lean_launch(const C3Group& h, int fam, int mode, unsigned grid, size_t lds, hipStream_t st);

template <int NP, int MF, int NF, int WM, int WN>
__global__ __launch_bounds__(256, 2) void conv3x3_split_kernel(C3Args p) {
  using G = Geo<NP>;
  constexpr int ROWB = G::ROWB, PST = G::PST, CPR = G::CPR, BROW = G::BROW, BLDS = G::BLDS;
  constexpr int BM = WM * MF * 16, BN = WN * NF * 16;
  constexpr int RPP = 256 / CPR;
  constexpr int PA = (BM + 2 * MAX_SW + 2 + RPP - 1) / RPP;
  constexpr int BPR = BROW / 16;
  constexpr int PB = (BN * BPR + 255) / 256;
  extern __shared__ __attribute__((aligned(16))) unsigned char smem[];
  const int na = p.na;
  const int arows = na * 32;
  unsigned char* At = smem;
  unsigned char* Bt = smem + (size_t)arows * ROWB;

  const int t = threadIdx.x, lane = t & 63, wave = t >> 6;
  const int i16 = lane & 15, g = lane >> 4;
  const int wave_m = wave % WM, wave_n = wave / WM;

  int bx, by;
  {
    const unsigned gx = gridDim.x, gy = gridDim.y, total = gx * gy;
    const unsigned lin = blockIdx.y * gx + blockIdx.x;
    const unsigned xcd = lin & 7, idx = lin >> 3, per = total >> 3, rem = total & 7;
    const unsigned L = xcd < rem ? xcd * (per + 1) + idx : rem * (per + 1) + (xcd - rem) * per + idx;
    bx = (int)(L / gy);
    by = (int)(L - (unsigned)bx * gy);
  }
  const int p0 = bx * BM, n0 = by * BN;
  const int halo = p.SW + 1;
  const int c4 = (t % CPR) * 4;
  const int prow = t / CPR;

  int goff[PA];
#pragma unroll
  for (int q = 0; q < PA; ++q) {
    const int row = prow + RPP * q;
    const int pp = p0 - halo + row;
    int o = row < arows ? -1 : -2;
    if (row < arows && pp >= 0 && pp < p.P) {
      const int n = fast_div(pp, p.ib_mul, p.ib_sh);
      const int rem = pp - n * p.IB;
      const int yy = fast_div(rem, p.sw_mul, p.sw_sh);
      const int xx = rem - yy * p.SW;
      if (n < p.N && yy >= 1 && xx >= 1 && xx <= p.W) o = ((n * p.H + yy - 1) * p.W + xx - 1) * p.Ci;
    }
    goff[q] = o;
  }

  f32x4 areg[PA], breg[PB];
  auto load_a = [&](int c0, int cw) {
#pragma unroll
    for (int q = 0; q < PA; ++q)
      if (RPP * q < arows) {
        const bool ok = goff[q] >= 0 && c4 < cw * 16;
        areg[q] = *reinterpret_cast<const f32x4*>(p.x + (ok ? goff[q] + c0 + c4 : 0));
      }
  };
  auto store_a = [&](int cw) {
#pragma unroll
    for (int q = 0; q < PA; ++q)
      if (RPP * q < arows && goff[q] != -2) {
        const int row = prow + RPP * q;
        const bool ok = goff[q] >= 0 && c4 < cw * 16;
        split_store<NP, PST>(At + (size_t)row * ROWB, c4, ok ? areg[q] : (f32x4){0.f, 0.f, 0.f, 0.f});
      }
  };
  int bsrc[PB], bdst[PB];
#pragma unroll
  for (int q = 0; q < PB; ++q) {
    const int id = t + 256 * q;
    const int nl = id / BPR, pc = id - nl * BPR;
    const bool ok = nl < BN;
    bsrc[q] = ok ? (n0 + nl) * BROW + pc * 16 : 0;
    bdst[q] = ok ? nl * BLDS + pc * 16 : (nl & 15) * BLDS + BROW + (t & 1) * 16;
  }
  const long step_bytes = (long)p.Co * BROW;
  auto load_b = [&](int gs) {
    const unsigned char* src = p.wp + gs * step_bytes;
#pragma unroll
    for (int q = 0; q < PB; ++q) breg[q] = *reinterpret_cast<const f32x4*>(src + bsrc[q]);
  };
  auto store_b = [&](int buf) {
    unsigned char* dst = Bt + (size_t)buf * BN * BLDS;
#pragma unroll
    for (int q = 0; q < PB; ++q) *reinterpret_cast<f32x4*>(dst + bdst[q]) = breg[q];
  };

  f32x4 acc[MF][NF];
#pragma unroll
  for (int mf = 0; mf < MF; ++mf)
#pragma unroll
    for (int nf = 0; nf < NF; ++nf) acc[mf][nf] = (f32x4){0.f, 0.f, 0.f, 0.f};

  const int nfull = NP == 2 ? p.Ci / CK : 0;
  const int ntail = NP == 2 ? ((p.Ci % CK) ? 1 : 0) : p.Ci / 16;
  const int nchunks = nfull + ntail, last_step = nfull * 9 + ntail * 5 - 1;
  const unsigned char* abase = At + (size_t)(wave_m * MF * 16 + i16) * ROWB + (g & 1) * 16;
  const unsigned char* bbase = Bt + (size_t)(wave_n * NF * 16 + i16) * BLDS + g * 16;
  const bool lowk = g < 2;
  int gs = 0, buf = 0;

  auto run_chunk = [&](auto cw_tag) {
    constexpr int CW = decltype(cw_tag)::value;
    constexpr int NS = CW == 2 ? 9 : 5;
#pragma unroll
    for (int s = 0; s < NS; ++s) {
      load_b(gs < last_step ? gs + 1 : last_step);
      const int tap0 = CW == 2 ? s : 2 * s;
      const int tap1 = CW == 2 ? s : (2 * s + 1 < 9 ? 2 * s + 1 : 2 * s);
      const int o0 = ((tap0 / 3) * p.SW + tap0 % 3) * ROWB;
      const int o1 = ((tap1 / 3) * p.SW + tap1 % 3) * ROWB + (CW == 2 ? 32 : 0);
      const unsigned char* ap = abase + (lowk ? o0 : o1);
      const unsigned char* bp = bbase + (size_t)buf * BN * BLDS;
      bf16x8 a[NP][MF], b[NP][NF];
#pragma unroll
      for (int nf = 0; nf < NF; ++nf)
#pragma unroll
        for (int q = 0; q < NP; ++q) b[q][nf] = *reinterpret_cast<const bf16x8*>(bp + nf * 16 * BLDS + q * 64);
#pragma unroll
      for (int mf = 0; mf < MF; ++mf)
#pragma unroll
        for (int q = 0; q < NP; ++q) a[q][mf] = *reinterpret_cast<const bf16x8*>(ap + mf * 16 * ROWB + q * PST);
#pragma unroll
      for (int mf = 0; mf < MF; ++mf) {
#define C3_MMA(qa, qb)                                                                                          \
  _Pragma("unroll") for (int nf = 0; nf < NF; ++nf) acc[mf][nf] =                                                \
      __builtin_amdgcn_mfma_f32_16x16x32_bf16(a[qa][mf], b[qb][nf], acc[mf][nf], 0, 0, 0);
        if constexpr (NP == 3) {
          C3_MMA(2, 0) C3_MMA(0, 2) C3_MMA(1, 1) C3_MMA(1, 0) C3_MMA(0, 1) C3_MMA(0, 0)
        } else {
          C3_MMA(1, 0) C3_MMA(0, 1) C3_MMA(0, 0)
        }
#undef C3_MMA
      }
      store_b(buf ^ 1);
      __syncthreads();
      buf ^= 1;
      ++gs;
    }
  };

  const int cw0 = nfull > 0 ? 2 : 1;
  load_a(0, cw0);
  load_b(0);
  store_a(cw0);
  store_b(0);
  if (nchunks > 1) load_a(cw0 * 16, nfull > 1 ? 2 : 1);
  __syncthreads();
  int c_next = cw0 * 16;
  for (int ch = 0; ch < nchunks; ++ch) {
// ... 322 lines not shown
  }
  split_store<2, 64>(reinterpret_cast<unsigned char*>(it.wprep) + rown * 128, c4, v);
}

__device__ __forceinline__ void prep3_piece(const float* __restrict__ w, unsigned char* __restrict__ out, int Kc, int Nc,
                                            int flip, long idx) {
  const int k4 = (int)(idx & 7);
  const long rown = idx >> 3;
  const int n = (int)(rown % Nc), step = (int)(rown / Nc);
  const int chunk = step / 5, s = step - chunk * 5;
  const int tap = 2 * s + (k4 >> 2);
  const int cc = chunk * 16 + (k4 & 3) * 4;
  f32x4 v = (f32x4){0.f, 0.f, 0.f, 0.f};
  if (tap < 9) {
    if (!flip) v = *reinterpret_cast<const f32x4*>(w + ((long)n * 9 + tap) * Kc + cc);
    else {
#pragma unroll
      for (int j = 0; j < 4; ++j) v[j] = w[((long)(cc + j) * 9 + (8 - tap)) * Nc + n];
    }
  }
  const int lane = (k4 >> 1) * 16 + (n & 15);
  unsigned char* dst = out + (((size_t)step * (Nc / 16) + (n >> 4)) * 3) * 1024 + lane * 16;
  split_store<3, 1024>(dst, (k4 & 1) * 4, v);
}
__global__ __launch_bounds__(256) void conv3x3_prep3_kernel(const float* __restrict__ w, unsigned char* __restrict__ out,
                                                            int Kc, int Nc, int flip, long items) {
  const long idx = (long)blockIdx.x * 256 + threadIdx.x;
  if (idx >= items) return;
  prep3_piece(w, out, Kc, Nc, flip, idx);
}

struct C3Plan { int MF, NF, WM, WN, BM, BN, na; size_t lds; bool single; };


static int c3_steps(int Kc, int np) { return np == 3 ? (Kc / 16) * 5 : (Kc / CK) * 9 + ((Kc % CK) ? 5 : 0); }

static bool c3_plan(int np, int N, int H, int W, int Ci, int Co, C3Plan* pl) {
  if (N <= 0 || H <= 0 || W <= 0 || Ci <= 0 || Co <= 0 || Ci % 16 != 0 || Co % 16 != 0 || c3_row_width(W) > MAX_SW) return false;
  const int rowb = np == 3 ? Geo<3>::ROWB : Geo<2>::ROWB, blds = np == 3 ? Geo<3>::BLDS : Geo<2>::BLDS;
  const long P = (long)N * (H + 1) * c3_row_width(W) + c3_row_width(W);
  int nf, wn;
  if (Co % 96 == 0) { nf = 3; wn = 2; }
  else if (Co % 48 == 0) { nf = 3; wn = 1; }
  else if (Co % 128 == 0) { nf = 4; wn = 2; }
  else if (Co % 64 == 0) { nf = 4; wn = 1; }
  else if (Co % 32 == 0) { nf = 2; wn = 1; }
  else { nf = 1; wn = 1; }
  if (np == 2 && Co % 96 == 0 && ((P + 127) / 128) * (Co / 96) < 320) { nf = 3; wn = 1; }
  bool small = false;
  if (np == 3 && Co % 32 == 0 && ((P + 127) / 128) * ((Co + 95) / 96) < 200) { nf = 2; wn = 1; small = true; }
  int wm = 4 / wn, bn = wn * nf * 16;
  int mf = 1;
  const int cand[2] = {4, 2};
  for (int i = (nf == 4 ? 1 : 0); i < 2; ++i) {
    const long blocks = ((P + wm * cand[i] * 16 - 1) / (wm * cand[i] * 16)) * (Co / bn);
    const long need = np == 3 ? (small ? 160 : 224) : 320;
    if (blocks >= need) { mf = cand[i]; break; }
  }
  bool single = false;
  if (np == 3 && nf == 3 && wn == 1 && Co == bn) {
    const long b8 = (P + 511) / 512;
    if (b8 > 256 && b8 <= 512) {
      mf = 8; single = true;
      if ((P + 447) / 448 <= 512) mf = 7;
    }
  }
  pl->MF = mf; pl->NF = nf; pl->WM = wm; pl->WN = wn; pl->BM = wm * mf * 16; pl->BN = bn; pl->single = single;
  pl->na = (pl->BM + 2 * c3_row_width(W) + 3 + 31) / 32;
  size_t stage = (size_t)4 * (mf >= 2 ? 2 : 1) * 16 * (nf * 16 + 4) * 4 + 4 * 128 * 4;
  if (np == 3 && stage < (size_t)C3_EPI_LDS) stage = C3_EPI_LDS;
  if (np == 3) {
    const int nb = single ? 1 : 2;
    while ((size_t)nb * pl->na * 32 * rowb < stage) ++pl->na;
    pl->lds = (size_t)nb * pl->na * 32 * rowb + (size_t)3 * Ci * sizeof(float);
  } else {
    while ((size_t)pl->na * 32 * rowb < stage) ++pl->na;
    pl->lds = (size_t)pl->na * 32 * rowb + (size_t)2 * pl->BN * blds;
  }
  return pl->lds <= 160 * 1024;
}

static bool c3_np_ok(int np) { return np == 2 || np == 3; }

template <int NP, int MF, int NF, int WM, int WN>
static int c3_launch(const C3Args& a, const C3Plan& pl, hipStream_t st) {
  static unsigned char attr_done[3][BUCTD_MAX_DEVICES] = {{0}};
  void (*fn)(C3Args);
  int variant = 0;
  if constexpr (NP == 3) {
    if (MF >= 7) fn = conv3x3_x6_kernel<MF, NF, WM, WN, false, false, 2>;
    else { fn = conv3x3_x6_kernel<MF, NF, WM, WN, true, true, 2>; variant = 2; }
  }
  else fn = conv3x3_split_kernel<NP, (MF > 4 ? 4 : MF), NF, WM, WN>;
  if (const int rc = buctd_raise_lds_limit(reinterpret_cast<const void*>(fn), 160 * 1024, attr_done[variant], "conv3x3 (split bf16)"))
    return rc;
  dim3 grid(ceil_div(a.P, pl.BM), a.Co / pl.BN);
  hipLaunchKernelGGL(fn, grid, dim3(256), pl.lds, st, a);
  BUCTD_CHECK_LAUNCH("buctd_conv3x3 (split bf16)");
  return BUCTD_OK;
}

template <int NP>
static int c3_dispatch(const C3Args& a, const C3Plan& pl, hipStream_t st, bool dry = false) {
#define C3_CASE(mf, nf, wm, wn) \
  if (pl.MF == mf && pl.NF == nf && pl.WN == wn) return dry ? BUCTD_OK : c3_launch<NP, mf, nf, wm, wn>(a, pl, st);
#define C3_MF(nf, wm, wn) C3_CASE(4, nf, wm, wn) C3_CASE(2, nf, wm, wn) C3_CASE(1, nf, wm, wn)
  if constexpr (NP == 3) { C3_CASE(8, 3, 4, 1) C3_CASE(7, 3, 4, 1) C3_CASE(8, 3, 2, 2) }
  C3_MF(1, 4, 1) C3_MF(2, 4, 1) C3_MF(3, 4, 1) C3_MF(3, 2, 2)
  C3_CASE(2, 4, 4, 1) C3_CASE(1, 4, 4, 1) C3_CASE(2, 4, 2, 2) C3_CASE(1, 4, 2, 2)
#undef C3_MF
#undef C3_CASE
  buctd_set_error("conv3x3 (split bf16): no kernel for MF=%d NF=%d WN=%d", pl.MF, pl.NF, pl.WN);
  return BUCTD_EINVAL;
}

static int c3_supported(int np, int N, int H, int W, int Ci, int Co) {
  C3Plan pl;
  return c3_np_ok(np) && c3_plan(np, N, H, W, Ci, Co, &pl) ? 1 : 0;
}

static int c3_stats_groups(int np, int N, int H, int W, int Ci, int Co, int* ngroups, int* rows_per_group) {
  C3Plan pl;
  BUCTD_CHECK_ARG(ngroups && rows_per_group && c3_np_ok(np) && c3_plan(np, N, H, W, Ci, Co, &pl),
                  "buctd_conv3x3_*_stats_groups: unsupported shape");
  const long P = (long)N * (H + 1) * c3_row_width(W) + c3_row_width(W);
  *ngroups = ceil_div(P, pl.BM) * pl.WM;
  *rows_per_group = pl.MF * 16;
  return BUCTD_OK;
}

static size_t c3_prep_bytes(int np, int Ci, int Co, int flip) {
  if (!c3_np_ok(np) || Ci <= 0 || Co <= 0 || Ci % 16 != 0 || Co % 16 != 0) return 0;
  const int Kc = flip ? Co : Ci, Nc = flip ? Ci : Co;
  return (size_t)c3_steps(Kc, np) * Nc * (np == 3 ? Geo<3>::BROW : Geo<2>::BROW);
}

static int c3_prep(int np, int Ci, int Co, const float* w, int flip, void* wprep, void* stream) {
  BUCTD_CHECK_ARG(w && wprep && c3_np_ok(np), "buctd_conv3x3_*_prep: null pointer");
  BUCTD_CHECK_ARG(Ci > 0 && Co > 0 && Ci % 16 == 0 && Co % 16 == 0, "buctd_conv3x3_*_prep: Ci=%d Co=%d must be multiples of 16",
                  Ci, Co);
  const int Kc = flip ? Co : Ci, Nc = flip ? Ci : Co;
  const long pieces = (long)c3_steps(Kc, np) * Nc * 8;
  if (np == 3)
    hipLaunchKernelGGL(conv3x3_prep3_kernel, dim3(ceil_div(pieces, 256)), dim3(256), 0, (hipStream_t)stream, w,
                       (unsigned char*)wprep, Kc, Nc, flip ? 1 : 0, pieces);
  else
    hipLaunchKernelGGL(conv3x3_prep_kernel, dim3(ceil_div(pieces, 256)), dim3(256), 0, (hipStream_t)stream, w,
                       (unsigned char*)wprep, Kc, Nc, flip ? 1 : 0, pieces);
  BUCTD_CHECK_LAUNCH("buctd_conv3x3_*_prep");
  return BUCTD_OK;
}

struct C3InBn { const float* gamma; const float* beta; int relu; };
struct C3BwdStat { const float* z; const float* y; const float* mean; const float* invstd; const float* gamma; const float* beta; long long* acc; };
struct C3Acc { long long* stats_acc; const buctd_bn_acc_in* in; };

static int c3_fill_shape(int np, int N, int H, int W, int Ci, int Co, C3Args& a, C3Plan& pl) {
  BUCTD_CHECK_ARG(c3_np_ok(np) && c3_plan(np, N, H, W, Ci, Co, &pl),
                  "buctd_conv3x3 (split bf16): unsupported shape N%d H%d W%d Ci%d Co%d", N, H, W, Ci, Co);
  a.N = N; a.H = H; a.W = W; a.Ci = Ci; a.Co = Co;
  a.SW = c3_row_width(W); a.IB = (H + 1) * a.SW;
  const long P = (long)N * a.IB + a.SW;
  BUCTD_CHECK_ARG(P < 2147483647L && (long)N * H * W * (Ci > Co ? Ci : Co) < 2147483647L,
                  "buctd_conv3x3 (split bf16): tensor too large");
  a.P = (int)P;
  a.na = pl.na;
  a.omap = 0; a.oH = H; a.oW = W; a.ost = 1; a.oy0 = a.ox0 = 0;
  a.col_major = (np == 3 && Co / pl.BN >= 2 && (size_t)c3_steps(Ci, 3) * Co * Geo<3>::BROW > ((size_t)3 << 20)) ? 1 : 0;
  magic_u32((unsigned)a.IB, &a.ib_mul, &a.ib_sh);
  magic_u32((unsigned)a.SW, &a.sw_mul, &a.sw_sh);
  return BUCTD_OK;
}

static int c3_fill(int np, int N, int H, int W, int Ci, int Co, const float* x, const void* wprep, const float* bias,
                   const float* scale, const float* shift, const float* residual, int relu, float* y,
                   float* stats_partials, int* stats_counts, const C3InBn* in_bn, const C3BwdStat* bst, const C3Acc* accs,
                   C3Args& a, C3Plan& pl) {
  BUCTD_CHECK_ARG(x && wprep && y, "buctd_conv3x3 (split bf16): null tensor pointer");
  if (const int rc = c3_fill_shape(np, N, H, W, Ci, Co, a, pl)) return rc;
  BUCTD_CHECK_ARG((scale == nullptr) == (shift == nullptr), "buctd_conv3x3 (split bf16): scale and shift go together");
  BUCTD_CHECK_ARG((stats_partials == nullptr) == (stats_counts == nullptr),
                  "buctd_conv3x3 (split bf16): stats partials and counts go together");
  a.x = x; a.wp = (const unsigned char*)wprep; a.out = y; a.bias = bias; a.scale = scale; a.shift = shift;
  a.res = residual; a.stats = stats_partials; a.counts = stats_counts;
  a.relu = relu;
  a.in_gamma = a.in_beta = nullptr;
  a.in_relu = 0;
  a.stats_acc = nullptr; a.bs_acc = nullptr;
  memset(&a.in_acc, 0, sizeof(a.in_acc));
  if (accs) {
    BUCTD_CHECK_ARG(np == 3, "buctd_conv3x3: statistics accumulators need the bf16x6 kernel");
    a.stats_acc = accs->stats_acc;
    if (accs->in && accs->in->acc) {
      const buctd_bn_acc_in& i = *accs->in;
      BUCTD_CHECK_ARG(in_bn && in_bn->gamma && in_bn->beta && i.rows > 0 && i.mean_out && i.invstd_out &&
                          (i.running_mean == nullptr) == (i.running_var == nullptr),
                      "buctd_conv3x3: input BatchNorm from an accumulator needs gamma, beta, rows, mean_out and invstd_out");
      a.in_gamma = in_bn->gamma; a.in_beta = in_bn->beta; a.in_relu = in_bn->relu;
      a.in_acc.acc = (const long long*)i.acc; a.in_acc.rows = (double)i.rows; a.in_acc.eps = i.eps; a.in_acc.momentum = i.momentum;
      a.in_acc.mean_out = i.mean_out; a.in_acc.invstd_out = i.invstd_out; a.in_acc.rmean = i.running_mean; a.in_acc.rvar = i.running_var;
    }
  }
  a.bs_z = a.bs_y = a.bs_mean = a.bs_invstd = a.bs_gamma = a.bs_beta = nullptr;
  if (bst && bst->acc) {
    BUCTD_CHECK_ARG(np == 3 && bst->z && bst->mean && bst->invstd && (bst->y || (bst->gamma && bst->beta)),
                    "buctd_conv3x3: the BatchNorm-backward by-product needs the bf16x6 kernel, z, mean, invstd and y or gamma + beta");
    a.bs_z = bst->z; a.bs_y = bst->y; a.bs_mean = bst->mean; a.bs_invstd = bst->invstd; a.bs_gamma = bst->gamma;
    a.bs_beta = bst->beta; a.bs_acc = bst->acc;
  }
  return BUCTD_OK;
}

static int c3_lean_mask(int m) {
  switch (m) {
    case C3M_STATS: case C3M_STATS | C3M_IN_BN: case C3M_BS_REBUILD: case C3M_RES | C3M_BS_Y: case C3M_RES: return m;
    default: return -1;
  }
}

static int c3_lean_mode(const C3Args& a) {
  if ((long)a.N * a.H * a.W * (a.Ci > a.Co ? a.Ci : a.Co) * 4 >= 2147483648L) return -1;
  if (a.bias || a.scale || a.shift || a.relu || a.stats || a.counts || a.omap) return -1;
  if (a.in_acc.acc && (!a.in_gamma || !a.in_beta)) return -1;
  int m = 0;
  if (a.in_acc.acc) m |= C3M_IN_BN;
  if (a.stats_acc) m |= C3M_STATS;
  if (a.res) m |= C3M_RES;
  if (a.bs_acc) m |= a.bs_y ? C3M_BS_Y : C3M_BS_REBUILD;
  return c3_lean_mask(m);
}

static int c3_group_variant(const C3Plan& pl, int* fam, bool general = false) {
  struct V { int mf, nf, wm, wn; };
  static const V f0[] = {{7, 3, 4, 1}, {4, 3, 2, 2}, {2, 2, 4, 1}, {4, 3, 4, 1}, {4, 2, 4, 1}};
  static const V f1[] = {{4, 2, 4, 1}, {1, 4, 4, 1}, {2, 2, 4, 1}, {1, 2, 4, 1}, {2, 4, 4, 1}, {2, 4, 2, 2}, {1, 3, 4, 1}, {2, 3, 4, 1}};
  for (int f = 0; f < 2; ++f) {
    if (*fam >= 0 && *fam != f) continue;
    const V* l = f ? f1 : f0;
    const int n = f ? (general ? 8 : 6) : 5;
    for (int i = 0; i < n; ++i)
      if (l[i].mf == pl.MF && l[i].nf == pl.NF && l[i].wm == pl.WM && l[i].wn == pl.WN) {
        *fam = f;
        return i;
      }
  }
  return -1;
}

struct C3Dry { int kernel, fam, variant, wgs; };

static int c3_group_launch(int n, const C3Args* a, const C3Plan* pl, hipStream_t stream, bool* done, C3Dry* dry = nullptr) {
  *done = false;
  int order[C3G_MAX];
  double cost[C3G_MAX];
  int lean = c3_lean_mode(a[0]);
  for (int k = 0; k < n; ++k) {
    cost[k] = (double)pl[k].BM * pl[k].BN * a[k].Ci;
    order[k] = k;
    if (c3_lean_mode(a[k]) != lean) lean = -1;
  }
  if (n == 1 && lean < 0) return BUCTD_OK;
  int fam = -1;
  bool ok = false;
  int var[C3G_MAX];
  for (int f = 0; f < 2 && !ok; ++f) {
    ok = true;
    for (int k = 0; k < n && ok; ++k) {
      fam = f;
      var[k] = c3_group_variant(pl[k], &fam, lean < 0);
      ok = var[k] >= 0;
    }
  }
  if (!ok) return BUCTD_OK;
  for (int i = 1; i < n; ++i)
    for (int j = i; j > 0 && cost[order[j]] > cost[order[j - 1]]; --j) { const int t = order[j]; order[j] = order[j - 1]; order[j - 1] = t; }
  C3Group h;
  h.nconv = n;
  size_t lds = 0;
  unsigned per_xcd = 0;
  for (int i = 0; i < n; ++i) {
    const int k = order[i];
    h.conv[i] = a[k];
    h.gx[i] = ceil_div(h.conv[i].P, pl[k].BM);
    h.gy[i] = h.conv[i].Co / pl[k].BN;
    h.tiles[i] = h.gx[i] * h.gy[i];
    h.variant[i] = var[k];
    const size_t l = pl[k].lds + (lean >= 0 ? (size_t)4 * pl[k].BN * sizeof(float) : 0);
    if (l > lds) lds = l;
    per_xcd += ((unsigned)h.tiles[i] + 7) >> 3;
  }
  for (int i = n; i < C3G_MAX; ++i) h.tiles[i] = h.gx[i] = h.gy[i] = h.variant[i] = 0;
  if (lds > 160 * 1024) return BUCTD_OK;
  *done = true;
  if (dry) { *dry = C3Dry{1, fam, h.variant[0], (int)(per_xcd * 8)}; return BUCTD_OK; }
  if (lean >= 0) return c3_lean_launch(h, fam, lean, per_xcd * 8, lds, stream);
  static unsigned char attr_done[2][BUCTD_MAX_DEVICES] = {{0}};
  void (*fn)(C3Group) = fam ? conv3x3_x6_group_kernel<1> : conv3x3_x6_group_kernel<0>;
  if (const int rc = buctd_raise_lds_limit(reinterpret_cast<const void*>(fn), 160 * 1024, attr_done[fam], "buctd_conv3x3_bf16x6_group"))
    return rc;
  hipLaunchKernelGGL(fn, dim3(per_xcd * 8), dim3(256), lds, stream, h);
  BUCTD_CHECK_LAUNCH("buctd_conv3x3_bf16x6_group");
  return BUCTD_OK;
}

static int c3_launch_one(const C3Args& a, const C3Plan& pl, hipStream_t stream, C3Dry* dry = nullptr) {
  bool done = false;
  const int rc = c3_group_launch(1, &a, &pl, stream, &done, dry);
  if (rc || done) return rc;
  if (dry) *dry = C3Dry{0, -1, -1, ceil_div(a.P, pl.BM) * (a.Co / pl.BN)};
  return c3_dispatch<3>(a, pl, stream, dry != nullptr);
}

static int c3_run(int np, int N, int H, int W, int Ci, int Co, const float* x, const void* wprep, const float* bias,
                  const float* scale, const float* shift, const float* residual, int relu, float* y,
                  float* stats_partials, int* stats_counts, void* stream, const C3InBn* in_bn = nullptr,
                  const C3BwdStat* bst = nullptr, const C3Acc* accs = nullptr) {
  C3Args a;
  C3Plan pl;
  const int rc = c3_fill(np, N, H, W, Ci, Co, x, wprep, bias, scale, shift, residual, relu, y, stats_partials, stats_counts,
                         in_bn, bst, accs, a, pl);
  if (rc) return rc;
  return np == 3 ? c3_launch_one(a, pl, (hipStream_t)stream) : c3_dispatch<2>(a, pl, (hipStream_t)stream);
}

extern "C" int buctd_conv3x3_bf16x3_supported(int N, int H, int W, int Ci, int Co) { return c3_supported(2, N, H, W, Ci, Co); }
extern "C" int buctd_conv3x3_bf16x3_stats_groups(int N, int H, int W, int Ci, int Co, int* ngroups, int* rows_per_group) {
  return c3_stats_groups(2, N, H, W, Ci, Co, ngroups, rows_per_group);
}
extern "C" size_t buctd_conv3x3_bf16x3_prep_bytes(int Ci, int Co, int flip) { return c3_prep_bytes(2, Ci, Co, flip); }
extern "C" int buctd_conv3x3_bf16x3_prep(int Ci, int Co, const float* w, int flip, void* wprep, void* stream) {
  return c3_prep(2, Ci, Co, w, flip, wprep, stream);
}
extern "C" int buctd_conv3x3_bf16x3_prep_batched(const buctd_c3_prep_item* items_device, int n, long total_pieces,
                                                 void* stream) {
  BUCTD_CHECK_ARG(items_device && n > 0 && total_pieces > 0, "buctd_conv3x3_bf16x3_prep_batched: bad argument");
  hipLaunchKernelGGL(conv3x3_prep_batched_kernel, dim3(ceil_div(total_pieces, 256)), dim3(256), 0, (hipStream_t)stream,
                     items_device, n, total_pieces);
  BUCTD_CHECK_LAUNCH("buctd_conv3x3_bf16x3_prep_batched");
  return BUCTD_OK;
}
extern "C" int buctd_conv3x3_bf16x3(int N, int H, int W, int Ci, int Co, const float* x, const void* wprep,
                                    const float* bias, const float* scale, const float* shift, const float* residual,
                                    int relu, float* y, float* stats_partials, int* stats_counts, void* stream) {
  return c3_run(2, N, H, W, Ci, Co, x, wprep, bias, scale, shift, residual, relu, y, stats_partials, stats_counts, stream);
}

extern "C" int buctd_conv3x3_bf16x6_supported(int N, int H, int W, int Ci, int Co) { return c3_supported(3, N, H, W, Ci, Co); }
extern "C" int buctd_conv3x3_bf16x6_stats_groups(int N, int H, int W, int Ci, int Co, int* ngroups, int* rows_per_group) {
  return c3_stats_groups(3, N, H, W, Ci, Co, ngroups, rows_per_group);
}
extern "C" size_t buctd_conv3x3_bf16x6_prep_bytes(int Ci, int Co, int flip) { return c3_prep_bytes(3, Ci, Co, flip); }
extern "C" int buctd_conv3x3_bf16x6_prep(int Ci, int Co, const float* w, int flip, void* wprep, void* stream) {
  return c3_prep(3, Ci, Co, w, flip, wprep, stream);
}
extern "C" int buctd_conv3x3_bf16x6(int N, int H, int W, int Ci, int Co, const float* x, const void* wprep,
                                    const float* bias, const float* scale, const float* shift, const float* residual,
                                    int relu, float* y, float* stats_partials, int* stats_counts, void* stream) {
  return c3_run(3, N, H, W, Ci, Co, x, wprep, bias, scale, shift, residual, relu, y, stats_partials, stats_counts, stream);
}

extern "C" int buctd_conv3x3_bf16x6_acc(int N, int H, int W, int Ci, int Co, const float* x, const void* wprep,
                                        const float* residual, int relu, float* y, void* stats_acc,
                                        const buctd_bn_acc_in* in_bn, const float* in_gamma, const float* in_beta, int in_relu,
                                        void* stream) {
  C3InBn b{in_gamma, in_beta, in_relu};
  C3Acc a{(long long*)stats_acc, in_bn};
  BUCTD_CHECK_ARG(!in_bn || in_bn->acc, "buctd_conv3x3_bf16x6_acc: in_bn without an accumulator");
  return c3_run(3, N, H, W, Ci, Co, x, wprep, nullptr, nullptr, nullptr, residual, relu, y, nullptr, nullptr, stream,
                in_bn ? &b : nullptr, nullptr, &a);
}
extern "C" int buctd_conv3x3_bf16x6_bnstat_acc(int N, int H, int W, int Ci, int Co, const float* x, const void* wprep,
                                               const float* residual, float* y, const float* bn_z, const float* bn_y,
                                               const float* bn_mean, const float* bn_invstd, const float* bn_gamma,
                                               const float* bn_beta, void* bn_acc, void* stream) {
  C3BwdStat b{bn_z, bn_y, bn_mean, bn_invstd, bn_gamma, bn_beta, (long long*)bn_acc};
  BUCTD_CHECK_ARG(bn_acc, "buctd_conv3x3_bf16x6_bnstat_acc: null accumulator");
  return c3_run(3, N, H, W, Ci, Co, x, wprep, nullptr, nullptr, nullptr, residual, 0, y, nullptr, nullptr, stream, nullptr,
                &b);
}

static int c3_group_fill(int n, const buctd_c3_conv* convs, C3Args* a, C3Plan* pl) {
  for (int k = 0; k < n; ++k) {
    const buctd_c3_conv& c = convs[k];
    C3InBn ib{c.in_gamma, c.in_beta, c.in_relu};
    C3BwdStat bs{c.bn_z, c.bn_y, c.bn_mean, c.bn_invstd, c.bn_gamma, c.bn_beta, (long long*)c.bn_acc};
    C3Acc ac{(long long*)c.stats_acc, c.in_bn};
    BUCTD_CHECK_ARG(!c.in_bn || c.in_bn->acc, "buctd_conv3x3_bf16x6_group: in_bn without an accumulator");
    const int rc = c3_fill(3, c.N, c.H, c.W, c.Ci, c.Co, c.x, c.wprep, nullptr, nullptr, nullptr, c.residual, c.relu, c.y,
                           nullptr, nullptr, c.in_bn ? &ib : nullptr, c.bn_acc ? &bs : nullptr, &ac, a[k], pl[k]);
    if (rc) return rc;
  }
  return BUCTD_OK;
}

extern "C" int buctd_conv3x3_bf16x6_group(int n, const buctd_c3_conv* convs, void* stream) {
  BUCTD_CHECK_ARG(n > 0 && n <= C3G_MAX && convs, "buctd_conv3x3_bf16x6_group: 1..%d convolutions", C3G_MAX);
  C3Args a[C3G_MAX];
  C3Plan pl[C3G_MAX];
  if (const int rc0 = c3_group_fill(n, convs, a, pl)) return rc0;
  bool done = false;
  const int rc = c3_group_launch(n, a, pl, (hipStream_t)stream, &done);
  if (rc || done) return rc;
  for (int k = 0; k < n; ++k)
    if (const int rc1 = c3_launch_one(a[k], pl[k], (hipStream_t)stream)) return rc1;
  return BUCTD_OK;
}

extern "C" int buctd_conv3x3_bf16x6_group_eval(int n, const buctd_c3_conv_eval* convs, void* stream) {
  BUCTD_CHECK_ARG(n > 0 && n <= C3G_MAX && convs, "buctd_conv3x3_bf16x6_group_eval: 1..%d convolutions", C3G_MAX);
  C3Args a[C3G_MAX];
  C3Plan pl[C3G_MAX];
  for (int k = 0; k < n; ++k) {
    const buctd_c3_conv_eval& c = convs[k];
    const int rc = c3_fill(3, c.N, c.H, c.W, c.Ci, c.Co, c.x, c.wprep, nullptr, c.scale, c.shift, c.residual, c.relu, c.y,
                           nullptr, nullptr, nullptr, nullptr, nullptr, a[k], pl[k]);
    if (rc) return rc;
  }
  bool done = false;
  const int rc = n > 1 ? c3_group_launch(n, a, pl, (hipStream_t)stream, &done) : BUCTD_OK;
  if (rc || done) return rc;
  for (int k = 0; k < n; ++k)
    if (const int rc1 = c3_dispatch<3>(a[k], pl[k], (hipStream_t)stream)) return rc1;
  return BUCTD_OK;
}

extern "C" int buctd_conv3x3_bf16x6_group_workgroups(int n, const buctd_c3_conv* convs) {
  BUCTD_CHECK_ARG(n > 0 && n <= C3G_MAX && convs, "buctd_conv3x3_bf16x6_group_workgroups: 1..%d convolutions", C3G_MAX);
  C3Args a[C3G_MAX];
  C3Plan pl[C3G_MAX];
  if (const int rc0 = c3_group_fill(n, convs, a, pl)) return rc0;
  bool done = false;
  C3Dry dry{};
  const int rc = c3_group_launch(n, a, pl, nullptr, &done, &dry);
  if (rc) return rc;
  return done ? dry.wgs : 0;
}

extern "C" int buctd_conv3x3_bf16x6_plan(int N, int H, int W, int Ci, int Co, int option_set, int* out) {
  BUCTD_CHECK_ARG(out && (option_set == -1 || c3_lean_mask(option_set) >= 0),
                  "buctd_conv3x3_bf16x6_plan: option set %d is not one of the train-mode sets (or -1)", option_set);
  static const float some = 0.f;
  const float* on = &some;
  C3Args a{};
  C3Plan pl;
  if (const int rc = c3_fill_shape(3, N, H, W, Ci, Co, a, pl)) return rc;
  if (option_set >= 0) {
    if (option_set & C3M_IN_BN) { a.in_acc.acc = (const long long*)on; a.in_gamma = a.in_beta = on; }
    if (option_set & C3M_STATS) a.stats_acc = (long long*)on;
    if (option_set & C3M_RES) a.res = on;
    if (option_set & (C3M_BS_REBUILD | C3M_BS_Y)) a.bs_acc = (long long*)on;
    if (option_set & C3M_BS_Y) a.bs_y = on;
  }
  C3Dry dry{};
  if (const int rc = c3_launch_one(a, pl, nullptr, &dry)) return rc;
  const int v[11] = {pl.MF, pl.NF, pl.WM, pl.WN, pl.single ? 1 : 0, a.col_major, dry.kernel, dry.fam, dry.variant, pl.BM, pl.BN};
  for (int i = 0; i < 11; ++i) out[i] = v[i];
  return BUCTD_OK;
}
```

### buctd_amd/csrc/conv3x3_lean.hip

```cpp
#include "c3_lean.h"

template <int FAM, int MODE>
__global__ __launch_bounds__(256, 2) void conv3x3_x6_lean_kernel(C3Group g_) {
  extern __shared__ __attribute__((aligned(16))) unsigned char smem[];
  const C3Group& g = *(const C3Group*)__builtin_amdgcn_kernarg_segment_ptr();
  const unsigned lin = blockIdx.x, xcd = lin & 7;
  unsigned idx = lin >> 3;
  int c = -1;
  unsigned L = 0;
  for (int k = 0; k < g.nconv; ++k) {
    const unsigned total = (unsigned)g.tiles[k], per = total >> 3, rem = total & 7;
    const unsigned mine = per + (xcd < rem ? 1u : 0u);
    if (idx < mine) {
      L = xcd < rem ? xcd * (per + 1) + idx : rem * (per + 1) + (xcd - rem) * per + idx;
      c = k;
      break;
    }
    idx -= mine;
  }
  if (c < 0) return;
  const C3Args& p = g.conv[c];
  int bx, by;
  if (p.col_major) {
    by = (int)(L / (unsigned)g.gx[c]);
    bx = (int)(L - (unsigned)by * g.gx[c]);
  } else {
    bx = (int)(L / (unsigned)g.gy[c]);
    by = (int)(L - (unsigned)bx * g.gy[c]);
  }
  const int v = g.variant[c];
  if constexpr (FAM == 0) {
    switch (v) {
      case 0: c3l_tile<7, 3, 4, 1, false, false, MODE>(p, smem, bx, by); break;
      case 1: c3l_tile<4, 3, 2, 2, true, true, MODE>(p, smem, bx, by); break;
      case 2: c3l_tile<2, 2, 4, 1, true, true, MODE>(p, smem, bx, by); break;
      case 3: c3l_tile<4, 3, 4, 1, true, true, MODE>(p, smem, bx, by); break;
      default: c3l_tile<4, 2, 4, 1, true, true, MODE>(p, smem, bx, by); break;
    }
  } else {
    switch (v) {
      case 0: c3l_tile<4, 2, 4, 1, true, true, MODE>(p, smem, bx, by); break;
      case 1: c3l_tile<1, 4, 4, 1, true, true, MODE>(p, smem, bx, by); break;
      case 2: c3l_tile<2, 2, 4, 1, true, true, MODE>(p, smem, bx, by); break;
      case 3: c3l_tile<1, 2, 4, 1, true, true, MODE>(p, smem, bx, by); break;
      case 4: c3l_tile<2, 4, 4, 1, true, true, MODE>(p, smem, bx, by); break;
      default: c3l_tile<2, 4, 2, 2, true, true, MODE>(p, smem, bx, by); break;
    }
  }
}

int c3_lean_launch(const C3Group& h, int fam, int mode, unsigned grid, size_t lds, hipStream_t st) {
  static unsigned char attr_done[2][5][BUCTD_MAX_DEVICES] = {{{0}}};
  void (*fn)(C3Group) = nullptr;
  int mi = -1;
#define C3L_PICK(i, m)                                                                               \
  if (mode == (m)) {                                                                                 \
    mi = i;                                                                                          \
    fn = fam ? conv3x3_x6_lean_kernel<1, (m)> : conv3x3_x6_lean_kernel<0, (m)>;                      \
  }
  C3L_PICK(0, C3M_STATS)
  C3L_PICK(1, C3M_STATS | C3M_IN_BN)
  C3L_PICK(2, C3M_BS_REBUILD)
  C3L_PICK(3, C3M_RES | C3M_BS_Y)
  C3L_PICK(4, C3M_RES)
#undef C3L_PICK
  if (!fn) {
    buctd_set_error("conv3x3 (bf16x6, train mode): no kernel for option set %d", mode);
    return BUCTD_EINVAL;
  }
  if (const int rc = buctd_raise_lds_limit(reinterpret_cast<const void*>(fn), 160 * 1024, attr_done[fam ? 1 : 0][mi],
                                           "conv3x3 (bf16x6, train mode)"))
    return rc;
  hipLaunchKernelGGL(fn, dim3(grid), dim3(256), lds, st, h);
  BUCTD_CHECK_LAUNCH("conv3x3 (bf16x6, train mode)");
  return BUCTD_OK;
}
```

### buctd_amd/csrc/conv_gather_x6.hip

```cpp
#include "c3_lean.h"
#include <string.h>

#define GC_MAXT 9
#define GC_TAB_OFF (56 * 1024)

struct GcClass {
  int ntaps, nhs, nsteps;
  int oy0, ox0;
  long wp_off;
  unsigned pdy, pdx;
};

struct GcArgs {
  C3Args e;
  const float* src;
  const unsigned char* wp;
  int SH, SWd, SC, ss, cpt;
  int ncls;
  GcClass cls[4];
};

template <int MF, int NF, int WM, int WN, int MODE>
__global__ __launch_bounds__(256, 2) void gconv_x6_kernel(GcArgs p) {
  constexpr int BM = WM * MF * 16, BN = WN * NF * 16, ROWB = 96, PST = 32, BROW = 192;
// ... 443 lines not shown
              const float d = v - piv[nf];
              s1[nf] += d;
              s2[nf] = __builtin_fmaf(d, d, s2[nf]);
            }
          }
        }
        __builtin_amdgcn_wave_barrier();
#pragma unroll
        for (int k = 0; k < 4; ++k) {
          const int item = lane + 64 * k, row = item >> 4, c4 = item & 15;
          const long grow = (long)blk * 32 + mf * 16 + row;
          f32x4 v = *reinterpret_cast<const f32x4*>(stg + row * R1_LD + c4 * 4);
          if (grow < p.rows) {
            const long o = grow * Co + cg * 64 + c4 * 4;
            if (p.res) v += *reinterpret_cast<const f32x4*>(p.res + o);
            *reinterpret_cast<f32x4*>(p.out + o) = v;
          }
        }
        __builtin_amdgcn_wave_barrier();
      }
    }
  }
  if (p.stats_acc) {
    __syncthreads();
    double2* exch = reinterpret_cast<double2*>(smem);
#pragma unroll
    for (int nf = 0; nf < NFT; ++nf) {
      const double pi = (double)piv[nf], nn = (double)nrows;
      double a1 = (double)s1[nf] + nn * pi, a2 = (double)s2[nf] + 2.0 * pi * (double)s1[nf] + nn * pi * pi;
      a1 += __shfl_xor(a1, 16, 64); a1 += __shfl_xor(a1, 32, 64);
      a2 += __shfl_xor(a2, 16, 64); a2 += __shfl_xor(a2, 32, 64);
      if (g == 0) exch[wave * Co + nf * 16 + i16] = make_double2(a1, a2);
    }
    __syncthreads();
    for (int c = t; c < Co; c += 512) {
      double a1 = 0.0, a2 = 0.0;
#pragma unroll
      for (int w = 0; w < 8; ++w) {
        const double2 v = exch[w * Co + c];
        a1 += v.x;
        a2 += v.y;
      }
      bnacc_add(p.stats_acc, Co, bnacc_shard(), c, a1, a2);
    }
  }
}

static bool r1_ok(int kind, long rows, int cin, int cout) {
  if (kind != 1 || cin % 32 || (cout != 64 && cout != 128 && cout != 256)) return false;
  const size_t lds = (size_t)(cin / 32) * cout * R1_WROW + (size_t)8 * R1_STG;
  return lds <= 150 * 1024 && (size_t)8 * cout * 16 <= (size_t)(cin / 32) * cout * R1_WROW && rows >= 65536;
}

static int r1_run(long rows, int cin, int cout, int nft, const float* x, const void* wprep, const float* bias, const float* residual,
                  float* out, long long* stats_acc, hipStream_t st, const char* who) {
  R1Args a;
  a.x = x; a.wp = (const unsigned char*)wprep; a.bias = bias; a.res = residual; a.out = out; a.stats_acc = stats_acc;
  a.rows = rows; a.Ci = cin; a.Co = cout; a.nblocks = (int)((rows + 31) / 32);
  const size_t lds = (size_t)(cin / 32) * cout * R1_WROW + (size_t)8 * R1_STG;
  static unsigned char done[3][BUCTD_MAX_DEVICES] = {{0}};
  void (*fn)(R1Args) = nft == 4 ? conv1x1_rows_x6_kernel<4> : nft == 8 ? conv1x1_rows_x6_kernel<8> : conv1x1_rows_x6_kernel<16>;
  if (const int rc = buctd_raise_lds_limit(reinterpret_cast<const void*>(fn), 160 * 1024, done[nft == 4 ? 0 : nft == 8 ? 1 : 2], who))
    return rc;
  int grid = 256;
  if (grid * 8 > a.nblocks) grid = (a.nblocks + 7) / 8;
  hipLaunchKernelGGL(fn, dim3(grid), dim3(512), lds, st, a);
  BUCTD_CHECK_LAUNCH(who);
  return BUCTD_OK;
}

enum { GCF_BIAS = 1, GCF_SCALE = 2, GCF_RELU = 4, GCF_PARTIALS = 8, GCF_ACC = 16, GCF_RES = 32, GCF_ALL = 63 };

struct GcRoute {
  int route;
  int Hg, Wg, SH, SWd, SC, nout;
  long rows;
  int P;
  GcPlan pl;
  int mode;
  int ncls;
  GcClass cls[4];
  int tiles, ncol;
  int nft, ksteps;
};

static int gc_route(int kind, int dir, int N, int H, int W, int Ci, int Co, int flags, const char* who, GcRoute* r) {
  memset(r, 0, sizeof(GcRoute));
  BUCTD_CHECK_ARG(gc_geo(kind, dir, N, H, W, Ci, Co, &r->Hg, &r->Wg, &r->SH, &r->SWd, &r->SC, &r->nout),
                  "%s: unsupported shape kind %d N%d H%d W%d Ci%d Co%d", who, kind, N, H, W, Ci, Co);
  BUCTD_CHECK_ARG(!(dir && (flags & (GCF_PARTIALS | GCF_ACC))), "%s: no statistics on the data gradient", who);
  const bool bias = flags & GCF_BIAS, scale = flags & GCF_SCALE, relu = flags & GCF_RELU, partials = flags & GCF_PARTIALS,
             acc = flags & GCF_ACC, res = flags & GCF_RES;
  const int SC = r->SC, nout = r->nout;
  r->rows = (long)N * H * W;
  if (!scale && !relu && !partials && r1_ok(kind, r->rows, SC, nout)) {
    r->route = 1;
    r->nft = nout / 16;
    r->ksteps = SC / 32;
    return BUCTD_OK;
  }
  const long P = (long)N * (r->Hg + 1) * (r->Wg + 2) + r->Wg + 2;
  r->P = (int)P;
  gc_plan(nout, P, &r->pl);
  const bool par = kind == 2 && dir;
  const int cpt = SC / 16;
  r->ncls = gc_ncls(kind, dir);
  long off = 0;
  int tr[GC_MAXT], ts[GC_MAXT];
  for (int c = 0; c < r->ncls; ++c) {
    GcClass& k = r->cls[c];
    int tdy[GC_MAXT], tdx[GC_MAXT];
    k.ntaps = gc_taps(kind, dir, c, tr, ts, tdy, tdx);
    for (int t = 0; t < k.ntaps; ++t) {
      k.pdy |= (unsigned)(tdy[t] + 1) << (2 * t);
      k.pdx |= (unsigned)(tdx[t] + 1) << (2 * t);
    }
    k.nhs = k.ntaps * cpt;
    k.nsteps = (k.nhs + 1) / 2;
    k.oy0 = par ? (c >> 1) : 0; k.ox0 = par ? (c & 1) : 0;
    k.wp_off = off;
    off += (long)gc_class_bytes(k.ntaps, SC, nout);
  }
  r->tiles = (int)((P + r->pl.BM - 1) / r->pl.BM);
  r->ncol = nout / r->pl.BN;
  r->mode = -1;
  if (!bias && !scale && !relu && !partials && !(acc && res) && (long)N * H * W * (Ci > Co ? Ci : Co) * 4 < 2147483648L)
    r->mode = acc ? C3M_STATS : res ? C3M_RES : 0;
  return BUCTD_OK;
}

static int gc_run(int kind, int dir, int N, int H, int W, int Ci, int Co, const float* src, const void* wprep, const float* bias,
                  const float* scale, const float* shift, const float* residual, int relu, float* out, float* stats_partials,
                  int* stats_counts, void* stream, const char* who, long long* stats_acc = nullptr) {
  BUCTD_CHECK_ARG(src && wprep && out, "%s: null tensor pointer", who);
  BUCTD_CHECK_ARG((scale == nullptr) == (shift == nullptr), "%s: scale and shift go together", who);
  BUCTD_CHECK_ARG((stats_partials == nullptr) == (stats_counts == nullptr), "%s: stats partials and counts go together", who);
  const int flags = (bias ? GCF_BIAS : 0) | (scale ? GCF_SCALE : 0) | (relu ? GCF_RELU : 0) | (stats_partials ? GCF_PARTIALS : 0) |
                    (stats_acc ? GCF_ACC : 0) | (residual ? GCF_RES : 0);
  GcRoute r;
  if (const int rc = gc_route(kind, dir, N, H, W, Ci, Co, flags, who, &r)) return rc;
  if (r.route == 1)
    return r1_run(r.rows, r.SC, r.nout, r.nft, src, wprep, bias, residual, out, stats_acc, (hipStream_t)stream, who);
  const GcPlan& pl = r.pl;
  GcArgs a;
  C3Args& e = a.e;
  e.x = nullptr; e.wp = nullptr; e.out = out; e.bias = bias; e.scale = scale; e.shift = shift; e.res = residual;
  e.stats = stats_partials; e.counts = stats_counts;
  e.N = N; e.H = r.Hg; e.W = r.Wg; e.Ci = r.SC; e.Co = r.nout;
  e.SW = r.Wg + 2; e.IB = (r.Hg + 1) * (r.Wg + 2);
  e.P = r.P;
  e.relu = relu; e.na = 0;
  e.in_gamma = e.in_beta = nullptr; e.in_relu = 0; e.col_major = 0;
  e.bs_z = e.bs_y = e.bs_mean = e.bs_invstd = e.bs_gamma = e.bs_beta = nullptr;
  e.stats_acc = stats_acc; e.bs_acc = nullptr;
  memset(&e.in_acc, 0, sizeof(e.in_acc));
  magic_u32((unsigned)e.IB, &e.ib_mul, &e.ib_sh);
  magic_u32((unsigned)e.SW, &e.sw_mul, &e.sw_sh);
  const bool par = kind == 2 && dir;
  e.omap = par ? 1 : 0; e.oH = H; e.oW = W; e.ost = par ? 2 : 1; e.oy0 = e.ox0 = 0;
  a.src = src; a.wp = (const unsigned char*)wprep;
  a.SH = r.SH; a.SWd = r.SWd; a.SC = r.SC; a.ss = (kind == 2 && !dir) ? 2 : 1; a.cpt = r.SC / 16;
  a.ncls = r.ncls;
  for (int c = 0; c < 4; ++c) a.cls[c] = r.cls[c];
  hipStream_t st = (hipStream_t)stream;
  if (pl.NF == 3 && pl.WM == 2) gc_launch<4, 3, 2, 2>(a, r.tiles, r.ncol, st, r.mode);
  else if (pl.NF == 4 && pl.WM == 2) gc_launch<4, 4, 2, 2>(a, r.tiles, r.ncol, st, r.mode);
  else if (pl.NF == 4) gc_launch<2, 4, 4, 1>(a, r.tiles, r.ncol, st, r.mode);
  else gc_launch<2, 3, 4, 1>(a, r.tiles, r.ncol, st, r.mode);
  BUCTD_CHECK_LAUNCH(who);
  return BUCTD_OK;
}

extern "C" int buctd_gconv_x6_plan(int kind, int dir, int N, int H, int W, int Ci, int Co, int flags, int* out) {
  BUCTD_CHECK_ARG(out && (dir == 0 || dir == 1) && flags >= 0 && flags <= GCF_ALL, "buctd_gconv_x6_plan: bad argument");
  BUCTD_CHECK_ARG(!(dir && (flags & ~GCF_RES)), "buctd_gconv_x6_plan: a data gradient carries the residual only (flags %d)", flags);
  BUCTD_CHECK_ARG(!((flags & GCF_ACC) && (flags & ~(GCF_ACC | GCF_BIAS))),
                  "buctd_gconv_x6_plan: the accumulator form carries the bias only (flags %d)", flags);
  GcRoute r;
  if (const int rc = gc_route(kind, dir, N, H, W, Ci, Co, flags, "buctd_gconv_x6_plan", &r)) return rc;
  int i = 0;
  out[i++] = r.route;
  out[i++] = r.pl.MF; out[i++] = r.pl.NF; out[i++] = r.pl.WM; out[i++] = r.pl.WN; out[i++] = r.pl.BM; out[i++] = r.pl.BN;
  out[i++] = r.route ? 0 : r.mode;
  out[i++] = r.ncls;
  for (int c = 0; c < 4; ++c) { out[i++] = r.cls[c].ntaps; out[i++] = r.cls[c].nhs; out[i++] = r.cls[c].nsteps; }
  out[i++] = r.tiles; out[i++] = r.ncol;
  out[i++] = r.nft; out[i++] = r.ksteps;
  return BUCTD_OK;
}

extern "C" int buctd_gconv_x6_fwd(int kind, int N, int H, int W, int Ci, int Co, const float* x, const void* wprep,
                                  const float* bias, const float* scale, const float* shift, const float* residual, int relu,
                                  float* y, float* stats_partials, int* stats_counts, void* stream) {
  return gc_run(kind, 0, N, H, W, Ci, Co, x, wprep, bias, scale, shift, residual, relu, y, stats_partials, stats_counts, stream,
                "buctd_gconv_x6_fwd");
}

extern "C" int buctd_gconv_x6_fwd_acc(int kind, int N, int H, int W, int Ci, int Co, const float* x, const void* wprep,
                                      const float* bias, float* y, void* stats_acc, void* stream) {
  BUCTD_CHECK_ARG(stats_acc, "buctd_gconv_x6_fwd_acc: null accumulator");
  return gc_run(kind, 0, N, H, W, Ci, Co, x, wprep, bias, nullptr, nullptr, nullptr, 0, y, nullptr, nullptr, stream,
                "buctd_gconv_x6_fwd_acc", (long long*)stats_acc);
}

extern "C" int buctd_gconv_x6_dgrad(int kind, int N, int H, int W, int Ci, int Co, const float* dy, const void* wprep,
                                    const float* residual, float* dx, void* stream) {
  return gc_run(kind, 1, N, H, W, Ci, Co, dy, wprep, nullptr, nullptr, nullptr, residual, 0, dx, nullptr, nullptr, stream,
                "buctd_gconv_x6_dgrad");
}
```

### include/buctd_hip.h

```cpp
#ifndef BUCTD_HIP_H
#define BUCTD_HIP_H
#include <stddef.h>
#include <stdint.h>

#ifdef __cplusplus
extern "C" {
#endif

int buctd_version(void);
const char* buctd_last_error(void);

typedef struct {
  int N, H, W, Ci;
  int Co, R, S;
  int stride, pad;
  int Ho, Wo;
} buctd_conv_desc;

int buctd_conv2d_fwd_thin(const buctd_conv_desc* d);
int buctd_conv2d_fwd(const buctd_conv_desc* d, const float* x, const float* w, const float* bias,
                     const float* scale, const float* shift, const float* residual, int relu, float* y,
                     float* stats_partials, void* stream);
int buctd_conv2d_dgrad(const buctd_conv_desc* d, const float* dy, const float* w, const float* bias, float* dx,
                       float* stats_partials, void* stream);
int buctd_conv2d_stats_groups(const buctd_conv_desc* d, int transposed, int* ngroups, int* rows_per_group);
size_t buctd_conv2d_wgrad_workspace(const buctd_conv_desc* d);
int buctd_conv2d_wgrad(const buctd_conv_desc* d, const float* x, const float* dy, float* dw, int accumulate,
                       void* workspace, size_t workspace_bytes, void* stream);
#define BUCTD_CONV_BIAS 1
#define BUCTD_CONV_SCALE 2
#define BUCTD_CONV_RESIDUAL 4
#define BUCTD_CONV_RELU 8
#define BUCTD_CONV_STATS 16
#define BUCTD_CONV_PLAN_INTS 11
int buctd_conv2d_plan(const buctd_conv_desc* d, int direction, int flags, int* out);

int buctd_conv3x3_bf16x6_supported(int N, int H, int W, int Ci, int Co);
int buctd_conv3x3_bf16x6_stats_groups(int N, int H, int W, int Ci, int Co, int* ngroups, int* rows_per_group);
size_t buctd_conv3x3_bf16x6_prep_bytes(int Ci, int Co, int flip);
int buctd_conv3x3_bf16x6_prep(int Ci, int Co, const float* w, int flip, void* wprep, void* stream);
int buctd_conv3x3_bf16x6(int N, int H, int W, int Ci, int Co, const float* x, const void* wprep, const float* bias,
                         const float* scale, const float* shift, const float* residual, int relu, float* y,
                         float* stats_partials, int* stats_counts, void* stream);
struct buctd_bn_acc_in_;
int buctd_conv3x3_bf16x6_acc(int N, int H, int W, int Ci, int Co, const float* x, const void* wprep, const float* residual,
                             int relu, float* y, void* stats_acc, const struct buctd_bn_acc_in_* in_bn, const float* in_gamma,
                             const float* in_beta, int in_relu, void* stream);
int buctd_conv3x3_bf16x6_bnstat_acc(int N, int H, int W, int Ci, int Co, const float* x, const void* wprep,
                                    const float* residual, float* y, const float* bn_z, const float* bn_y,
                                    const float* bn_mean, const float* bn_invstd, const float* bn_gamma, const float* bn_beta,
                                    void* bn_acc, void* stream);
typedef struct {
  int N, H, W, Ci, Co;
  const float* x;
  const void* wprep;
  const float* residual;
  int relu;
  float* y;
  void* stats_acc;
  const struct buctd_bn_acc_in_* in_bn;
  const float *in_gamma, *in_beta;
  int in_relu;
  const float *bn_z, *bn_y, *bn_mean, *bn_invstd, *bn_gamma, *bn_beta;
  void* bn_acc;
} buctd_c3_conv;
int buctd_conv3x3_bf16x6_group(int n, const buctd_c3_conv* convs, void* stream);
typedef struct {
  int N, H, W, Ci, Co;
  const float* x;
  const void* wprep;
  const float *scale, *shift;
  const float* residual;
  int relu;
  float* y;
} buctd_c3_conv_eval;
int buctd_conv3x3_bf16x6_group_eval(int n, const buctd_c3_conv_eval* convs, void* stream);
int buctd_conv3x3_bf16x6_group_workgroups(int n, const buctd_c3_conv* convs);
int buctd_conv3x3_bf16x6_plan(int N, int H, int W, int Ci, int Co, int option_set, int* out);
int buctd_conv3x3_bf16x3_supported(int N, int H, int W, int Ci, int Co);
int buctd_conv3x3_bf16x3_stats_groups(int N, int H, int W, int Ci, int Co, int* ngroups, int* rows_per_group);
size_t buctd_conv3x3_bf16x3_prep_bytes(int Ci, int Co, int flip);
int buctd_conv3x3_bf16x3_prep(int Ci, int Co, const float* w, int flip, void* wprep, void* stream);
typedef struct {
  const float* w;
  void* wprep;
  int Ci, Co, flip, reserved;
  long piece_begin;
} buctd_c3_prep_item;
int buctd_conv3x3_bf16x3_prep_batched(const buctd_c3_prep_item* items_device, int n, long total_pieces, void* stream);
int buctd_conv3x3_bf16x3(int N, int H, int W, int Ci, int Co, const float* x, const void* wprep, const float* bias,
                         const float* scale, const float* shift, const float* residual, int relu, float* y,
                         float* stats_partials, int* stats_counts, void* stream);

int buctd_conv3x3_wgrad_bf16x6_supported(int N, int H, int W, int Ci, int Co);
int buctd_conv3x3_wgrad_bf16x6_plan(int N, int H, int W, int Ci, int Co, int* out);
size_t buctd_conv3x3_wgrad_bf16x6_workspace(int N, int H, int W, int Ci, int Co);
int buctd_conv3x3_wgrad_bf16x6(int N, int H, int W, int Ci, int Co, const float* x, const float* dy, float* dw,
                               int accumulate, void* workspace, size_t workspace_bytes, void* stream);
int buctd_conv3x3_wgrad_bf16x6_bnin(int N, int H, int W, int Ci, int Co, const float* x, const float* dy, float* dw,
                                    int accumulate, const float* x_mean, const float* x_invstd, const float* x_gamma,
                                    const float* x_beta, int x_relu, void* workspace, size_t workspace_bytes,
                                    void* stream);
typedef struct {
  int N, H, W, Ci, Co;
  const float *x, *dy;
  float* dw;
  int accumulate;
  const float *x_mean, *x_invstd, *x_gamma, *x_beta;
  int x_relu;
  void* workspace;
  size_t workspace_bytes;
} buctd_wg3_conv;
size_t buctd_conv3x3_wgrad_bf16x6_group_workspace(int n, int N, int H, int W, int Ci, int Co);
int buctd_conv3x3_wgrad_bf16x6_group(int n, const buctd_wg3_conv* convs, void* stream);
int buctd_conv3x3_wgrad_bf16x6_group_workgroups(int n, const buctd_wg3_conv* convs);
int buctd_conv3x3_wgrad_bf16x3_supported(int N, int H, int W, int Ci, int Co);
size_t buctd_conv3x3_wgrad_bf16x3_workspace(int N, int H, int W, int Ci, int Co);
int buctd_conv3x3_wgrad_bf16x3(int N, int H, int W, int Ci, int Co, const float* x, const float* dy, float* dw,
                               int accumulate, void* workspace, size_t workspace_bytes, void* stream);

typedef struct {
  int batch, M, N, K;
  int a_layout;
  int b_layout;
  int lda, ldb, ldc;
  long stride_a, stride_b, stride_c;
  int Kc; long group_stride_a, group_stride_bk;
  int Nc; long group_stride_bn, group_stride_c;
  float alpha;
  int bias_axis;
} buctd_matmul_desc;
size_t buctd_matmul_workspace(const buctd_matmul_desc* d);
int buctd_matmul(const buctd_matmul_desc* d, const float* A, const float* B, const float* bias, float* C,
                 void* workspace, size_t workspace_bytes, void* stream);
#define BUCTD_MATMUL_PLAN_INTS 8
int buctd_matmul_plan(const buctd_matmul_desc* d, const void* A, const void* B, int* out);

int buctd_bn_finalize(const float* partials, const int* group_counts, int ngroups, int rows_per_group, long rows,
                      int C, float eps, float momentum, float* mean, float* invstd, float* running_mean,
                      float* running_var, void* stream);
int buctd_bn_stats(const float* z, long rows, int C, float* partials, int* ngroups, int* rows_per_group,
                   void* stream);
int buctd_bn_stats_groups(long rows, int C, int* ngroups, int* rows_per_group);
int buctd_bn_apply(const float* z, const float* mean, const float* invstd, const float* gamma, const float* beta,
                   const float* residual, int relu, float* y, long rows, int C, void* stream);
size_t buctd_bn_bwd_workspace(long rows, int C);
int buctd_bn_bwd(const float* dy, const float* y, const float* z, const float* mean, const float* invstd,
                 const float* gamma, const float* beta, int relu, long rows, int C, float* dz, float* dres,
                 float* dgamma, float* dbeta, int accumulate, void* workspace, size_t workspace_bytes, void* stream);
int buctd_bn_bwd_from_partials(const float* dy, const float* y, const float* z, const float* mean, const float* invstd,
                               const float* gamma, const float* beta, int relu, long rows, int C, const float* part,
                               int nparts, float* dz, float* dres, float* dgamma, float* dbeta, int accumulate,
                               void* workspace, size_t workspace_bytes, void* stream);
size_t buctd_bn_acc_bytes(int C);
typedef struct buctd_bn_acc_in_ {
  const void* acc;
  long rows;
  float eps, momentum;
  float *mean_out, *invstd_out;
  float *running_mean, *running_var;
} buctd_bn_acc_in;
int buctd_bn_apply_acc(const float* z, const buctd_bn_acc_in* st, const float* gamma, const float* beta,
                       const float* residual, int relu, float* y, long rows, int C, void* stream);
int buctd_bn_bwd_acc(const float* dy, const float* y, const float* z, const float* mean, const float* invstd,
                     const float* gamma, const float* beta, int relu, long rows, int C, float* dz, float* dres,
                     float* dgamma, float* dbeta, int accumulate, void* acc, int acc_ready, void* stream);
typedef struct {
  const float* z;
  buctd_bn_acc_in st;
  const float *gamma, *beta, *residual;
  int relu;
  float* y;
  long rows;
  int C;
} buctd_bn_apply_item;
int buctd_bn_apply_acc_group(int n, const buctd_bn_apply_item* items, void* stream);
typedef struct {
  const float *dy, *y, *z, *mean, *invstd, *gamma, *beta;
  int relu;
  long rows;
  int C;
  float *dz, *dres, *dgamma, *dbeta;
  int accumulate;
  void* acc;
  int acc_ready;
} buctd_bn_bwd_item;
int buctd_bn_bwd_acc_group(int n, const buctd_bn_bwd_item* items, void* stream);
int buctd_bn_fold(const float* gamma, const float* beta, const float* running_mean, const float* running_var,
                  float eps, int C, float* scale, float* shift, void* stream);

int buctd_add(const float* a, const float* b, float* out, long n, int relu, void* stream);
int buctd_add_n(const float* const* terms, int n, float* out, long count, void* stream);
int buctd_mul(const float* a, const float* b, float* out, long n, void* stream);
int buctd_scale(const float* x, const float* dev_scalar, float alpha, float* out, long n, void* stream);
int buctd_copy_channels(const float* src, long rows, int Cs, int cs0, float* dst, int Cd, int cd0, int Cc,
                        void* stream);
int buctd_add_bcast(const float* a, const float* v, float* out, long batch, long n, void* stream);
int buctd_batch_sum(const float* x, long batch, long n, float* out, int accumulate, void* stream);
int buctd_relu_bwd(const float* dy, const float* y, float* dx, long n, void* stream);
size_t buctd_colsum_workspace(long rows, int C);
int buctd_colsum(const float* x, long rows, int C, float* out, int accumulate, void* workspace,
                 size_t workspace_bytes, void* stream);
int buctd_nchw_to_nhwc(const float* x, int N, int Ctot, int c0, int Cc, int H, int W, float* y, void* stream);
int buctd_nhwc_to_nchw(const float* x, int N, int C, int H, int W, float* y, void* stream);
int buctd_fuse_sum(const float* const* terms, const int* shifts, int nterms, int N, int H, int W, int C, int relu,
                   float* out, void* stream);
int buctd_fuse_sum_bwd(const float* dy, const float* y, int shift, int N, int H, int W, int C, float* g,
                       void* stream);
int buctd_resize_bilinear(const float* x, int N, int Ctot, int c0, int Cc, int H, int W, int Ho, int Wo, float* y,
                          void* stream);
int buctd_maxpool3x3s2_fwd(const float* x, int N, int H, int W, int C, float* y, int32_t* idx, void* stream);
int buctd_maxpool3x3s2_bwd(const float* dy, const int32_t* idx, int N, int H, int W, int C, float* dx,
                           void* stream);

int buctd_softmax_dropout_fwd(const float* s, long rows, int L, float scale, float p_drop, uint64_t seed, float* p,
                              float* pd, void* stream);
int buctd_softmax_dropout_bwd(const float* dpd, const float* p, long rows, int L, float scale, float p_drop,
                              uint64_t seed, float* ds, void* stream);
int buctd_softmax_dropout_fwd_dseed(const float* s, long rows, int L, float scale, float p_drop, const uint64_t* seed,
                                    float* p, float* pd, void* stream);
int buctd_softmax_dropout_bwd_dseed(const float* dpd, const float* p, long rows, int L, float scale, float p_drop,
                                    const uint64_t* seed, float* ds, void* stream);
int buctd_attn_smallqk_supported(int T, int R4, int C);
#define BUCTD_ATTN_SMALLQK_PLAN_INTS 7
int buctd_attn_smallqk_plan(int T, int R4, int C, int flag, float p_drop, int dseed, int* out);
int buctd_attn_smallqk_fwd(int B, int T, int R4, int C, const float* q, const float* k, const float* v, float scale,
                           float p_drop, uint64_t seed, int bf16x3, float* out, float* m, float* linv, void* stream);
int buctd_attn_smallqk_bwd(int B, int T, int R4, int C, const float* q, const float* k, const float* v,
                           const float* o, const float* dout, const float* m, const float* linv, float scale,
                           float p_drop, uint64_t seed, int bf16x3, float* dq, float* dk, float* dv,
                           float* dvec_workspace, void* stream);
int buctd_attn_smallqk_fwd_dseed(int B, int T, int R4, int C, const float* q, const float* k, const float* v, float scale,
                                 float p_drop, const uint64_t* seed, int bf16x3, float* out, float* m, float* linv,
                                 void* stream);
int buctd_attn_smallqk_bwd_dseed(int B, int T, int R4, int C, const float* q, const float* k, const float* v,
                                 const float* o, const float* dout, const float* m, const float* linv, float scale,
                                 float p_drop, const uint64_t* seed, int bf16x3, float* dq, float* dk, float* dv,
                                 float* dvec_workspace, void* stream);
int buctd_dropout(const float* x, float* y, long n, float p_drop, uint64_t seed, void* stream);
int buctd_dropout_dseed(const float* x, float* y, long n, float p_drop, const uint64_t* seed, void* stream);
int buctd_dropout_seed_fill(uint64_t* table, int n, uint64_t base, uint64_t counter0, void* stream);
int buctd_layernorm_fwd(const float* x, const float* gamma, const float* beta, long rows, int C, float eps, float* y,
                        float* mean, float* invstd, void* stream);
int buctd_add_layernorm_fwd(const float* a, const float* b, const float* gamma, const float* beta, long rows, int C, float eps,
                            float* sum_out, float* y, float* mean, float* invstd, void* stream);
size_t buctd_layernorm_bwd_workspace(long rows, int C);
int buctd_layernorm_bwd(const float* dy, const float* x, const float* mean, const float* invstd, const float* gamma,
                        long rows, int C, float* dx, float* dgamma, float* dbeta, int accumulate, void* workspace,
                        size_t workspace_bytes, void* stream);

int buctd_joints_mse(const float* pred, const float* gt, const float* w, int N, int K, int HW, float* loss,
                     float* grad, float gscale, void* workspace, size_t workspace_bytes, void* stream);
#define BUCTD_OHKM_MAX_JOINTS 64
size_t buctd_joints_ohkm_mse_workspace(int N, int K);
int buctd_joints_ohkm_mse(const float* pred, const float* gt, const float* w, int N, int K, int HW, int topk, float* loss,
                          float* grad, float gscale, void* workspace, size_t workspace_bytes, void* stream);
int buctd_argmax_decode(const float* hm, int rows, int H, int W, float* preds, float* maxvals, int32_t* idx,
                        void* stream);
int buctd_argmax_decode_refined(const float* hm, int rows, int H, int W, float* preds, float* maxvals, int32_t* idx,
                                float* quarter, void* stream);
#define BUCTD_DARK_MAX_PIXELS 8000
int buctd_argmax_decode_dark(const float* hm, int rows, int H, int W, float* preds, float* maxvals, int32_t* idx,
                             float* offset, void* stream);
int buctd_gaussian_target(const float* joints, const float* vis, int B, int K, int Hh, int Wh, float stride_x,
                          float stride_y, float sigma, float* target, float* weight, void* stream);
size_t buctd_cond_render_workspace(int B, int Cc, int H, int W);
int buctd_cond_render(const float* joints, int js, const float* colors, int B, int K, int Cc, int H, int W,
                      int truncate, float* cond, void* workspace, size_t workspace_bytes, void* stream);
int buctd_flipback_avg(const float* a, const float* b, const int32_t* perm, int N, int K, int H, int W, int shift,
                       float* out, void* stream);

int buctd_gconv_x6_supported(int kind, int N, int H, int W, int Ci, int Co, int dir);
size_t buctd_gconv_x6_prep_bytes(int kind, int Ci, int Co, int dir);
int buctd_gconv_x6_prep(int kind, int Ci, int Co, const float* w, int dir, void* wprep, void* stream);
size_t buctd_gconv_x6_prep_item_bytes(void);
int buctd_gconv_x6_prep_item(int kind, int Ci, int Co, const float* w, int dir, void* wprep, void* item_host);
int buctd_gconv_x6_prep_batched(const void* items_device, int n, void* stream);
int buctd_gconv_x6_stats_groups(int kind, int N, int H, int W, int Ci, int Co, int* ngroups, int* rows_per_group);
int buctd_gconv_x6_fwd(int kind, int N, int H, int W, int Ci, int Co, const float* x, const void* wprep, const float* bias,
                       const float* scale, const float* shift, const float* residual, int relu, float* y,
                       float* stats_partials, int* stats_counts, void* stream);
int buctd_gconv_x6_fwd_acc(int kind, int N, int H, int W, int Ci, int Co, const float* x, const void* wprep, const float* bias,
                           float* y, void* stats_acc, void* stream);
int buctd_gconv_x6_dgrad(int kind, int N, int H, int W, int Ci, int Co, const float* dy, const void* wprep,
                         const float* residual, float* dx, void* stream);
int buctd_gconv_x6_plan(int kind, int dir, int N, int H, int W, int Ci, int Co, int flags, int* out);
int buctd_gconv_wgrad_x6_supported(int kind, int N, int H, int W, int Ci, int Co);
int buctd_gconv_wgrad_x6_plan(int kind, int N, int H, int W, int Ci, int Co, int* out);
size_t buctd_gconv_wgrad_x6_workspace(int kind, int N, int H, int W, int Ci, int Co);
int buctd_gconv_wgrad_x6(int kind, int N, int H, int W, int Ci, int Co, const float* x, const float* dy, float* dw,
                         int accumulate, void* workspace, size_t workspace_bytes, void* stream);

typedef struct {
  int N, H, W, C;
  const float* x;
  const void *w1_fwd, *w2_fwd;
  const void *w1_bwd, *w2_bwd;
  const float *gamma1, *beta1, *gamma2, *beta2;
  float *running_mean1, *running_var1, *running_mean2, *running_var2;
  float eps1, momentum1, eps2, momentum2;
  float *z1, *z2, *y;
  void* acc;
  float* stat;
} buctd_basic_block;
typedef struct {
  const float* dy;
  float *dz2, *dres, *dy1, *dz1;
  float* dx;
  float *dw1, *dw2, *dgamma1, *dbeta1, *dgamma2, *dbeta2;
  int acc_w1, acc_w2, acc_bn1, acc_bn2;
  void* bn_acc;
  void* wg_ws; size_t wg_ws_bytes;
} buctd_basic_block_grads;
int buctd_basic_chain_fwd_train(int n, const buctd_basic_block* blocks, void* stream);
int buctd_basic_chain_bwd(int n, const buctd_basic_block* blocks, const buctd_basic_block_grads* grads, void* stream,
                          void* side_stream);

int buctd_basic_branches_fwd_train(int nb, int n, const buctd_basic_block* blocks, void* stream);
int buctd_basic_branches_bwd(int nb, int n, const buctd_basic_block* blocks, const buctd_basic_block_grads* grads, void* stream,
                             void* side_stream);

int buctd_stream_fork(void* from, void* to);

int buctd_x6_image_dims(int V, int K, int role, int* Vpad, int* Kpad);
size_t buctd_x6_image_bytes(int V, int K, int role);
int buctd_x6_image(const float* src, int V, int K, int vg, long vgs, long vs, int kg, long kgs, long ks, int role,
                   void* image, void* stream);
int buctd_x6_gemm(int M, int N, int K, const void* a_image, const void* b_image, const float* bias, int bias_axis,
                  float alpha, float* C, long ldc, int Nc, long gsc, void* stream);
int buctd_x6_gemm_plan(int M, int N, int K, int* out);
int buctd_x6_gemm_tile(int lin, int gx, int gy, int row_major, int* bx, int* by);
int buctd_x6_image_path(const float* src, int V, int K, int vg, long vgs, long vs, int kg, long kgs, long ks, int role,
                        int v, int k0, int* vector);

int buctd_adam_step(float* p, const float* g, float* m, float* v, long n, float lr, float beta1, float beta2,
                    float eps, int step, float gscale, void* stream);
int buctd_sgd_step(float* p, const float* g, float* momentum_buf, long n, float lr, float momentum, float weight_decay,
                   int nesterov, int first_step, float gscale, void* stream);
int buctd_adam_step_dscale(float* p, const float* g, float* m, float* v, long n, float lr, float beta1, float beta2,
                           float eps, int step, float gscale, const float* coef, void* stream);
int buctd_sgd_step_dscale(float* p, const float* g, float* momentum_buf, long n, float lr, float momentum,
                          float weight_decay, int nesterov, int first_step, float gscale, const float* coef, void* stream);

#define BUCTD_STEP_MAX_GROUPS 16
#define BUCTD_STEP_CHUNK 16384
typedef struct {
  long start;
  int len;
  int group;
} buctd_step_chunk;
typedef struct {
  float lr, beta1, beta2, eps, weight_decay;
  int decoupled;
  int step;
} buctd_adam_group;
typedef struct {
  float lr, momentum, weight_decay;
  int nesterov;
} buctd_sgd_group;
long buctd_step_chunks(const long* runs, const int* run_group, int nruns, buctd_step_chunk* out);
int buctd_adam_step_groups(float* p, const float* g, float* m, float* v, const buctd_step_chunk* chunks_device, long nchunks,
                           const buctd_adam_group* groups, int ngroups, float gscale, const float* coef, void* stream);
int buctd_sgd_step_groups(float* p, const float* g, float* buf, const buctd_step_chunk* chunks_device, long nchunks,
                          const buctd_sgd_group* groups, int ngroups, float gscale, const float* coef, void* stream);

#define BUCTD_GRAD_SUMSQ_CHUNK 8192
size_t buctd_grad_sumsq_workspace(const long* runs, int nruns);
int buctd_grad_sumsq(const float* g, const long* runs, int nruns, double* sumsq, void* workspace, size_t workspace_bytes,
                     void* stream);
int buctd_grad_clip_coef(const double* sumsq, double gscale, double max_norm, float* coef, float* total_norm, void* stream);
int buctd_grad_segment_stats(const float* g, const long* spans, int P, double* abs_mean, double* norm, void* stream);

int buctd_ema_update(const float* p, float* avg, long n, float w, void* stream);
typedef struct {
  const float* src;
  float* avg;
  long n;
} buctd_avg_item;
int buctd_ema_update_tensors(const buctd_avg_item* items_device, int nitems, float w, void* stream);
int buctd_swap(float* a, float* b, long n, void* stream);

typedef struct buctd_mha_args {
  int B, T, h, dh;
  const float* q; const float* k; const float* v;
  int ldq, ldk, ldv;
  float* out; int ldo;
  float* lse;
  float scale, p_drop;
  const float* dout; int lddo;
  float* dq; float* dk; float* dv;
  int lddq, lddk, lddv;
} buctd_mha_args;
int buctd_mha_heads_fwd_supported(int T, int h, int dh);
int buctd_mha_heads_fwd(const buctd_mha_args* a, void* stream);
int buctd_mha_heads_fwd_bf16x6(const buctd_mha_args* a, void* stream);
size_t buctd_mha_fwd_bf16x6_workspace(int B, int T, int d);
int buctd_mha_heads_fwd_bf16x6_ws(const buctd_mha_args* a, void* workspace, size_t workspace_bytes, void* stream);
int buctd_mha_heads_train_supported(int T, int h, int dh);
int buctd_mha_heads_fwd_train(const buctd_mha_args* a, uint64_t seed, void* stream);
size_t buctd_mha_heads_bwd_workspace(int B, int h, int T);
int buctd_mha_heads_bwd(const buctd_mha_args* a, uint64_t seed, void* workspace, size_t workspace_bytes, void* stream);
int buctd_mha_heads_fwd_train_dseed(const buctd_mha_args* a, const uint64_t* seed, void* stream);
int buctd_mha_heads_bwd_dseed(const buctd_mha_args* a, const uint64_t* seed, void* workspace, size_t workspace_bytes,
                              void* stream);

typedef struct buctd_attn_rows_args {
  int B, T, h, dh, R;
  const float* q; const float* k;
  int ldq, ldk;
  const int* rows;
  float scale;
  float* out;
  float* out_heads;
} buctd_attn_rows_args;
int buctd_attn_rows_supported(int T, int h, int dh);
int buctd_attn_rows(const buctd_attn_rows_args* a, void* stream);

typedef struct {
  const unsigned char* src;
  int H, W;
  int flip;
  int rx, ry, rw, rh;
  double m[6];
} buctd_warp_item;
int buctd_warp_affine_norm(const buctd_warp_item* items_device, int B, int dst_h, int dst_w, const float* mean3,
                           const float* std3, float* out, long out_batch_stride, unsigned char* crop_u8, void* stream);
int buctd_cond_render_into(const float* joints, int js, const float* colors, int B, int K, int Cc, int H, int W,
                           int truncate, float* cond, long cond_batch_stride, void* workspace, size_t workspace_bytes,
                           void* stream);
int buctd_cond_geometry(const double* synth, const double* cond_vis, const buctd_warp_item* items_device,
                        const int* pair_device, int B, int K, double* out_joints, double* out_vis, float* out_trunc,
                        void* stream);
int buctd_cond_mirror(const double* cond_joints, int joint_stride, const double* cond_vis, const int* pair_device, int B,
                      int K, int width, float* out, void* stream);
int buctd_mirror_rows(const float* in, long in_batch_stride, float* out, long out_batch_stride, const int32_t* perm,
                      int B, int channel0, int channels, int H, int W, void* stream);
typedef struct {
  const float* coords;
  const float* maxvals;
  const float* offset;
  float* center;
  float* scale;
  double* box_score;
  buctd_warp_item* items;
  float* cond_trunc;
  double* cond_joints;
  int32_t* status;
  float* hist_preds;
  double* hist_score;
  double* hist_box_score;
  double* hist_keypoint_score;
  float* hist_center;
  float* hist_scale;
  int B, K, pass, passes;
  int heatmap_w, heatmap_h, crop_w, crop_h;
  double margin, aspect_ratio, in_vis_thre, scale_thre;
} buctd_refine_args;
int buctd_refine_step(const buctd_refine_args* a, void* stream);
#define BUCTD_GEOM_HAS_BBOX 1
#define BUCTD_GEOM_USE_BU_BBOX 2
#define BUCTD_GEOM_HALF_BODY 4
#define BUCTD_GEOM_FLIP 8
typedef struct {
  const double* joints;
  const double* joints_vis;
  const double* cond;
  const double* cond_vis;
  const float* center;
  const float* scale;
  const double* bbox;
  const float* half_body;
  const double* draws;
  const int32_t* bbox_draws;
// ... 140 lines not shown
```

Measured before the change: 515.8 images/s.

## Fold ReLU mask into dgrad epilogue so chained BN backward skips y and dres

In chained basic-block backward, the dgrad conv epilogue now applies the next block's ReLU mask (taken from bn_y) before storing dx, so the stored gradient is already masked. The following BN backward then runs in a new DY_MASKED mode that reads neither y nor writes dres, and the next dgrad uses dy directly as its residual. The aim is to cut one full activation read and one gradient write per chained block. The cost is a new lean-kernel specialisation and extra mask logic in the epilogue, plus a helper that reports which blocks run with pre-masked gradients.

```diff
diff --git a/buctd_amd/_C.py b/buctd_amd/_C.py
--- a/buctd_amd/_C.py
+++ b/buctd_amd/_C.py
@@ -37,7 +37,8 @@
                 [(n, C.c_void_p) for n in ("x", "wprep", "residual")] + [("relu", C.c_int)] +
                 [(n, C.c_void_p) for n in ("y", "stats_acc")] + [("in_bn", C.POINTER(BnAccIn))] +
                 [(n, C.c_void_p) for n in ("in_gamma", "in_beta")] + [("in_relu", C.c_int)] +
-                [(n, C.c_void_p) for n in ("bn_z", "bn_y", "bn_mean", "bn_invstd", "bn_gamma", "bn_beta", "bn_acc")])
+                [(n, C.c_void_p) for n in ("bn_z", "bn_y", "bn_mean", "bn_invstd", "bn_gamma", "bn_beta", "bn_acc")] +
+                [("bn_mask_out", C.c_int)])
 
 
 class C3ConvEval(C.Structure):
@@ -208,6 +209,7 @@
     "buctd_bn_bwd_acc": (_I, [_P, _P, _P, _P, _P, _P, _P, _I, _L, _I, _P, _P, _P, _P, _I, _P, _I, _P]),
     "buctd_conv3x3_bf16x6_acc": (_I, [_I] * 5 + [_P, _P, _P, _I, _P, _P, C.POINTER(BnAccIn), _P, _P, _I, _P]),
     "buctd_conv3x3_bf16x6_bnstat_acc": (_I, [_I] * 5 + [_P] * 12),
+    "buctd_conv3x3_bf16x6_bnstat_acc_masked": (_I, [_I] * 5 + [_P] * 12),
     "buctd_gconv_x6_fwd_acc": (_I, [_I] * 6 + [_P] * 6),
     "buctd_conv3x3_bf16x6_group": (_I, [_I, C.POINTER(C3Conv), _P]),
     "buctd_conv3x3_bf16x6_group_eval": (_I, [_I, C.POINTER(C3ConvEval), _P]),
@@ -228,6 +230,7 @@
     "buctd_basic_branches_bwd": (_I, [_I, _I, C.POINTER(BasicBlockDesc), C.POINTER(BasicBlockGrads), _P, _P]),
     "buctd_basic_chain_fwd_train": (_I, [_I, C.POINTER(BasicBlockDesc), _P]),
     "buctd_basic_chain_bwd": (_I, [_I, C.POINTER(BasicBlockDesc), C.POINTER(BasicBlockGrads), _P, _P]),
+    "buctd_basic_row_dy_masked": (_I, [_I, _I, C.POINTER(BasicBlockDesc), C.POINTER(BasicBlockGrads), C.POINTER(C.c_int)]),
     "buctd_x6_image_dims": (_I, [_I, _I, _I, _P, _P]),
     "buctd_x6_image_bytes": (C.c_size_t, [_I, _I, _I]),
     "buctd_x6_image": (_I, [_P, _I, _I, _I, _L, _L, _I, _L, _L, _I, _P, _P]),
diff --git a/buctd_amd/csrc/block.hip b/buctd_amd/csrc/block.hip
--- a/buctd_amd/csrc/block.hip
+++ b/buctd_amd/csrc/block.hip
@@ -70,6 +70,9 @@
 }
 static int issue_dgrad(bool group, int n, const buctd_c3_conv* c, void* s) {
   if (group) return buctd_conv3x3_bf16x6_group(n, c, s);
+  if (c->bn_acc && c->bn_mask_out)
+    return buctd_conv3x3_bf16x6_bnstat_acc_masked(c->N, c->H, c->W, c->Ci, c->Co, c->x, c->wprep, c->residual, c->y, c->bn_z,
+                                                  c->bn_y, c->bn_mean, c->bn_invstd, c->bn_gamma, c->bn_beta, c->bn_acc, s);
   if (c->bn_acc)
     return buctd_conv3x3_bf16x6_bnstat_acc(c->N, c->H, c->W, c->Ci, c->Co, c->x, c->wprep, c->residual, c->y, c->bn_z, c->bn_y,
                                            c->bn_mean, c->bn_invstd, c->bn_gamma, c->bn_beta, c->bn_acc, s);
@@ -147,7 +150,10 @@
       const buctd_basic_block_grads& G = grads[b * n + k];
       chain[b] = k > 0 && bn2_sums_chain(&B, &G);
       bi[b] = buctd_bn_bwd_item{G.dy, B.y, B.z2, mean2_of(B), invstd2_of(B), B.gamma2, nullptr, 1, (long)B.N * B.H * B.W, B.C,
-                                G.dz2, G.dres, G.dgamma2, G.dbeta2, G.acc_bn2, acc2_of(G.bn_acc, B.C), ready[b] ? 1 : 0};
+                                G.dz2, G.dres, G.dgamma2, G.dbeta2, G.acc_bn2, acc2_of(G.bn_acc, B.C), 0};
+      if (ready[b]) {
+        bi[b].y = nullptr; bi[b].relu = BUCTD_BN_RELU_DY_MASKED; bi[b].dres = nullptr; bi[b].acc_ready = 1;
+      }
     }
     BLK_TRY(issue_bn_bwd(group, nb, bi, stream));
     BLK_TRY(stream_fork(main_s, side_s, who));
@@ -186,14 +192,16 @@
     for (int b = 0; b < nb; ++b) {
       const buctd_basic_block& B = blocks[b * n + k];
       const buctd_basic_block_grads& G = grads[b * n + k];
+      const bool dy_masked = ready[b];
       ready[b] = chain[b];
       if (!G.dx) continue;
       buctd_c3_conv& c = cv[m++] = c3_of(B);
-      c.x = G.dz1; c.wprep = B.w1_bwd; c.residual = G.dres; c.y = G.dx;
+      c.x = G.dz1; c.wprep = B.w1_bwd; c.residual = dy_masked ? G.dy : G.dres; c.y = G.dx;
       if (chain[b]) {
         const buctd_basic_block& Bp = blocks[b * n + k - 1];
         c.bn_z = Bp.z2; c.bn_y = Bp.y; c.bn_mean = mean2_of(Bp); c.bn_invstd = invstd2_of(Bp); c.bn_gamma = Bp.gamma2;
         c.bn_acc = acc2_of(grads[b * n + k - 1].bn_acc, B.C);
+        c.bn_mask_out = 1;
       }
     }
     if (m) BLK_TRY(issue_dgrad(group, m, cv, stream));
@@ -228,6 +236,15 @@
   return row_bwd(true, "buctd_basic_branches_bwd", nb, n, blocks, grads, stream, side_stream);
 }
 
+extern "C" int buctd_basic_row_dy_masked(int nb, int n, const buctd_basic_block* blocks, const buctd_basic_block_grads* grads,
+                                         int* out) {
+  BUCTD_CHECK_ARG(nb > 0 && nb <= BR_MAX && n > 0 && blocks && grads && out, "buctd_basic_row_dy_masked: bad argument");
+  for (int b = 0; b < nb; ++b)
+    for (int k = 0; k < n; ++k)
+      out[b * n + k] = (k + 1 < n && bn2_sums_chain(&blocks[b * n + k + 1], &grads[b * n + k + 1])) ? 1 : 0;
+  return BUCTD_OK;
+}
+
 extern "C" int buctd_stream_fork(void* from, void* to) {
   return stream_fork((hipStream_t)from, (hipStream_t)to, "buctd_stream_fork");
 }
diff --git a/buctd_amd/csrc/bn.hip b/buctd_amd/csrc/bn.hip
--- a/buctd_amd/csrc/bn.hip
+++ b/buctd_amd/csrc/bn.hip
@@ -936,9 +936,12 @@
   BUCTD_CHECK_ARG(it.dy && it.z && it.mean && it.invstd && it.gamma && it.dz && it.acc && it.rows > 0 && it.C > 0 && it.C % 4 == 0 &&
                       it.C / 4 <= 256,
                   "%s: bad argument (C must be a multiple of 4, <= 1024)", who);
-  BUCTD_CHECK_ARG(!it.relu || it.y || it.beta, "%s: relu backward needs the forward output, or beta to rebuild its sign", who);
+  const bool dy_masked = it.relu == BUCTD_BN_RELU_DY_MASKED;
+  BUCTD_CHECK_ARG(!dy_masked || (it.acc_ready && !it.y && !it.dres),
+                  "%s: a pre-masked upstream gradient comes with its sums (acc_ready), without y and without dres", who);
+  BUCTD_CHECK_ARG(dy_masked || !it.relu || it.y || it.beta, "%s: relu backward needs the forward output, or beta to rebuild its sign", who);
   a.dy = it.dy; a.y = it.y; a.z = it.z; a.mean = it.mean; a.invstd = it.invstd; a.gamma = it.gamma; a.beta = it.beta;
-  a.acc = (long long*)it.acc; a.relu = it.relu; a.rows = it.rows; a.C = it.C;
+  a.acc = (long long*)it.acc; a.relu = dy_masked ? 0 : it.relu; a.rows = it.rows; a.C = it.C;
   *nb = bwd2_blocks(it.rows, &a.rows_per_block);
   a.inv_rows = 1.0f / (float)it.rows;
   a.dz = it.dz; a.dres = it.dres; a.dgamma = it.dgamma; a.dbeta = it.dbeta; a.accumulate = it.accumulate;
diff --git a/buctd_amd/csrc/c3_common.h b/buctd_amd/csrc/c3_common.h
--- a/buctd_amd/csrc/c3_common.h
+++ b/buctd_amd/csrc/c3_common.h
@@ -50,6 +50,7 @@
   const float* bs_invstd;
   const float* bs_gamma;
   const float* bs_beta;
+  int bs_mask_out;
   long long* stats_acc;
   long long* bs_acc;
   BnAccFwd in_acc;
@@ -262,6 +263,11 @@
 #pragma unroll
           for (int j = 0; j < 4; ++j) v[j] = fmaxf(v[j], 0.f);
         }
+        if (has_y && p.bs_mask_out) {
+          const f32x4 yy = pre_y[ps & 1][k];
+#pragma unroll
+          for (int j = 0; j < 4; ++j) v[j] = yy[j] > 0.f ? v[j] : 0.f;
+        }
         *reinterpret_cast<f32x4*>(p.out + off + n) = v;
         if (bs_on) {
           const f32x4 zz = pre_z[ps & 1][k];
diff --git a/buctd_amd/csrc/c3_lean.h b/buctd_amd/csrc/c3_lean.h
--- a/buctd_amd/csrc/c3_lean.h
+++ b/buctd_amd/csrc/c3_lean.h
@@ -1,7 +1,7 @@
 #pragma once
 #include "c3_common.h"
 
-enum { C3M_IN_BN = 1, C3M_STATS = 2, C3M_RES = 4, C3M_BS_REBUILD = 8, C3M_BS_Y = 16 };
+enum { C3M_IN_BN = 1, C3M_STATS = 2, C3M_RES = 4, C3M_BS_REBUILD = 8, C3M_BS_Y = 16, C3M_MASK_OUT = 32 };
 
 #define C3_OOB 0x80000000u
 __device__ __forceinline__ __amdgpu_buffer_rsrc_t c3_rsrc(const void* ptr, unsigned bytes) {
@@ -23,7 +23,9 @@
                                              int n0) {
   constexpr bool STATS = (MODE & C3M_STATS) != 0, RES = (MODE & C3M_RES) != 0;
   constexpr bool BSR = (MODE & C3M_BS_REBUILD) != 0, BSY = (MODE & C3M_BS_Y) != 0, BS = BSR || BSY;
+  constexpr bool MASK_OUT = (MODE & C3M_MASK_OUT) != 0;
   static_assert(!(STATS && BS), "c3l_epilogue: forward statistics and backward sums never meet in one launch");
+  static_assert(!MASK_OUT || BSY, "c3l_epilogue: the masked store takes its mask from bs_y");
   const int t = threadIdx.x, lane = t & 63;
   const int wave = __builtin_amdgcn_readfirstlane(t >> 6);
   const int i16 = lane & 15, g = lane >> 4;
@@ -141,6 +143,11 @@
     for (int k = 0; k < NI; ++k) {
       const bool ok = off[k] != C3_OOB;
       if constexpr (RES) v[k] += pre_r[ps & 1][k];
+      if constexpr (MASK_OUT) {
+        const f32x4 ym = pre_y[ps & 1][k];
+#pragma unroll
+        for (int j = 0; j < 4; ++j) v[k][j] = ym[j] > 0.f ? v[k][j] : 0.f;
+      }
       c3_bstore(r_out, off[k] + colb + c4_k[k] * 16, v[k]);
       if constexpr (STATS) {
         f32x4 d = v[k] - pq[k % NACC];
diff --git a/buctd_amd/csrc/conv3x3.hip b/buctd_amd/csrc/conv3x3.hip
--- a/buctd_amd/csrc/conv3x3.hip
+++ b/buctd_amd/csrc/conv3x3.hip
@@ -1,7 +1,7 @@
 #include "c3_common.h"
 #include <string.h>
 
-enum { C3M_IN_BN = 1, C3M_STATS = 2, C3M_RES = 4, C3M_BS_REBUILD = 8, C3M_BS_Y = 16 };
+enum { C3M_IN_BN = 1, C3M_STATS = 2, C3M_RES = 4, C3M_BS_REBUILD = 8, C3M_BS_Y = 16, C3M_MASK_OUT = 32 };
 int c3_lean_launch(const C3Group& h, int fam, int mode, unsigned grid, size_t lds, hipStream_t st);
 
 template <int NP, int MF, int NF, int WM, int WN>
@@ -630,7 +630,7 @@
 }
 
 struct C3InBn { const float* gamma; const float* beta; int relu; };
-struct C3BwdStat { const float* z; const float* y; const float* mean; const float* invstd; const float* gamma; const float* beta; long long* acc; };
+struct C3BwdStat { const float* z; const float* y; const float* mean; const float* invstd; const float* gamma; const float* beta; long long* acc; int mask_out; };
 struct C3Acc { long long* stats_acc; const buctd_bn_acc_in* in; };
 
 static int c3_fill_shape(int np, int N, int H, int W, int Ci, int Co, C3Args& a, C3Plan& pl) {
@@ -680,18 +680,22 @@
     }
   }
   a.bs_z = a.bs_y = a.bs_mean = a.bs_invstd = a.bs_gamma = a.bs_beta = nullptr;
+  a.bs_mask_out = 0;
+  BUCTD_CHECK_ARG(!(bst && bst->mask_out) || (bst->acc && bst->y),
+                  "buctd_conv3x3: the masked store needs the BatchNorm-backward by-product with bn_y");
   if (bst && bst->acc) {
     BUCTD_CHECK_ARG(np == 3 && bst->z && bst->mean && bst->invstd && (bst->y || (bst->gamma && bst->beta)),
                     "buctd_conv3x3: the BatchNorm-backward by-product needs the bf16x6 kernel, z, mean, invstd and y or gamma + beta");
     a.bs_z = bst->z; a.bs_y = bst->y; a.bs_mean = bst->mean; a.bs_invstd = bst->invstd; a.bs_gamma = bst->gamma;
-    a.bs_beta = bst->beta; a.bs_acc = bst->acc;
+    a.bs_beta = bst->beta; a.bs_acc = bst->acc; a.bs_mask_out = bst->mask_out ? 1 : 0;
   }
   return BUCTD_OK;
 }
 
 static int c3_lean_mask(int m) {
   switch (m) {
-    case C3M_STATS: case C3M_STATS | C3M_IN_BN: case C3M_BS_REBUILD: case C3M_RES | C3M_BS_Y: case C3M_RES: return m;
+    case C3M_STATS: case C3M_STATS | C3M_IN_BN: case C3M_BS_REBUILD: case C3M_RES | C3M_BS_Y: case C3M_RES:
+    case C3M_RES | C3M_BS_Y | C3M_MASK_OUT: return m;
     default: return -1;
   }
 }
@@ -705,6 +709,7 @@
   if (a.stats_acc) m |= C3M_STATS;
   if (a.res) m |= C3M_RES;
   if (a.bs_acc) m |= a.bs_y ? C3M_BS_Y : C3M_BS_REBUILD;
+  if (a.bs_mask_out) m |= C3M_MASK_OUT;
   return c3_lean_mask(m);
 }
 
@@ -851,8 +856,17 @@
                                                const float* residual, float* y, const float* bn_z, const float* bn_y,
                                                const float* bn_mean, const float* bn_invstd, const float* bn_gamma,
                                                const float* bn_beta, void* bn_acc, void* stream) {
-  C3BwdStat b{bn_z, bn_y, bn_mean, bn_invstd, bn_gamma, bn_beta, (long long*)bn_acc};
+  C3BwdStat b{bn_z, bn_y, bn_mean, bn_invstd, bn_gamma, bn_beta, (long long*)bn_acc, 0};
   BUCTD_CHECK_ARG(bn_acc, "buctd_conv3x3_bf16x6_bnstat_acc: null accumulator");
+  return c3_run(3, N, H, W, Ci, Co, x, wprep, nullptr, nullptr, nullptr, residual, 0, y, nullptr, nullptr, stream, nullptr,
+                &b);
+}
+extern "C" int buctd_conv3x3_bf16x6_bnstat_acc_masked(int N, int H, int W, int Ci, int Co, const float* x, const void* wprep,
+                                                      const float* residual, float* y, const float* bn_z, const float* bn_y,
+                                                      const float* bn_mean, const float* bn_invstd, const float* bn_gamma,
+                                                      const float* bn_beta, void* bn_acc, void* stream) {
+  C3BwdStat b{bn_z, bn_y, bn_mean, bn_invstd, bn_gamma, bn_beta, (long long*)bn_acc, 1};
+  BUCTD_CHECK_ARG(bn_acc && bn_y, "buctd_conv3x3_bf16x6_bnstat_acc_masked: null accumulator or bn_y");
   return c3_run(3, N, H, W, Ci, Co, x, wprep, nullptr, nullptr, nullptr, residual, 0, y, nullptr, nullptr, stream, nullptr,
                 &b);
 }
@@ -861,7 +875,8 @@
   for (int k = 0; k < n; ++k) {
     const buctd_c3_conv& c = convs[k];
     C3InBn ib{c.in_gamma, c.in_beta, c.in_relu};
-    C3BwdStat bs{c.bn_z, c.bn_y, c.bn_mean, c.bn_invstd, c.bn_gamma, c.bn_beta, (long long*)c.bn_acc};
+    C3BwdStat bs{c.bn_z, c.bn_y, c.bn_mean, c.bn_invstd, c.bn_gamma, c.bn_beta, (long long*)c.bn_acc, c.bn_mask_out};
+    BUCTD_CHECK_ARG(!c.bn_mask_out || (c.bn_acc && c.bn_y), "buctd_conv3x3_bf16x6_group: bn_mask_out needs bn_acc and bn_y");
     C3Acc ac{(long long*)c.stats_acc, c.in_bn};
     BUCTD_CHECK_ARG(!c.in_bn || c.in_bn->acc, "buctd_conv3x3_bf16x6_group: in_bn without an accumulator");
     const int rc = c3_fill(3, c.N, c.H, c.W, c.Ci, c.Co, c.x, c.wprep, nullptr, nullptr, nullptr, c.residual, c.relu, c.y,
@@ -928,6 +943,7 @@
     if (option_set & C3M_RES) a.res = on;
     if (option_set & (C3M_BS_REBUILD | C3M_BS_Y)) a.bs_acc = (long long*)on;
     if (option_set & C3M_BS_Y) a.bs_y = on;
+    if (option_set & C3M_MASK_OUT) a.bs_mask_out = 1;
   }
   C3Dry dry{};
   if (const int rc = c3_launch_one(a, pl, nullptr, &dry)) return rc;
diff --git a/buctd_amd/csrc/conv3x3_lean.hip b/buctd_amd/csrc/conv3x3_lean.hip
--- a/buctd_amd/csrc/conv3x3_lean.hip
+++ b/buctd_amd/csrc/conv3x3_lean.hip
@@ -50,7 +50,7 @@
 }
 
 int c3_lean_launch(const C3Group& h, int fam, int mode, unsigned grid, size_t lds, hipStream_t st) {
-  static unsigned char attr_done[2][5][BUCTD_MAX_DEVICES] = {{{0}}};
+  static unsigned char attr_done[2][6][BUCTD_MAX_DEVICES] = {{{0}}};
   void (*fn)(C3Group) = nullptr;
   int mi = -1;
 #define C3L_PICK(i, m)                                                                               \
@@ -63,6 +63,7 @@
   C3L_PICK(2, C3M_BS_REBUILD)
   C3L_PICK(3, C3M_RES | C3M_BS_Y)
   C3L_PICK(4, C3M_RES)
+  C3L_PICK(5, C3M_RES | C3M_BS_Y | C3M_MASK_OUT)
 #undef C3L_PICK
   if (!fn) {
     buctd_set_error("conv3x3 (bf16x6, train mode): no kernel for option set %d", mode);
diff --git a/buctd_amd/csrc/conv_gather_x6.hip b/buctd_amd/csrc/conv_gather_x6.hip
--- a/buctd_amd/csrc/conv_gather_x6.hip
+++ b/buctd_amd/csrc/conv_gather_x6.hip
@@ -619,7 +619,7 @@
   e.relu = relu; e.na = 0;
   e.in_gamma = e.in_beta = nullptr; e.in_relu = 0; e.col_major = 0;
   e.bs_z = e.bs_y = e.bs_mean = e.bs_invstd = e.bs_gamma = e.bs_beta = nullptr;
-  e.stats_acc = stats_acc; e.bs_acc = nullptr;
+  e.stats_acc = stats_acc; e.bs_acc = nullptr; e.bs_mask_out = 0;
   memset(&e.in_acc, 0, sizeof(e.in_acc));
   magic_u32((unsigned)e.IB, &e.ib_mul, &e.ib_sh);
   magic_u32((unsigned)e.SW, &e.sw_mul, &e.sw_sh);
diff --git a/include/buctd_hip.h b/include/buctd_hip.h
--- a/include/buctd_hip.h
+++ b/include/buctd_hip.h
@@ -50,6 +50,10 @@
                                     const float* residual, float* y, const float* bn_z, const float* bn_y,
                                     const float* bn_mean, const float* bn_invstd, const float* bn_gamma, const float* bn_beta,
                                     void* bn_acc, void* stream);
+int buctd_conv3x3_bf16x6_bnstat_acc_masked(int N, int H, int W, int Ci, int Co, const float* x, const void* wprep,
+                                           const float* residual, float* y, const float* bn_z, const float* bn_y,
+                                           const float* bn_mean, const float* bn_invstd, const float* bn_gamma,
+                                           const float* bn_beta, void* bn_acc, void* stream);
 typedef struct {
   int N, H, W, Ci, Co;
   const float* x;
@@ -63,6 +67,7 @@
   int in_relu;
   const float *bn_z, *bn_y, *bn_mean, *bn_invstd, *bn_gamma, *bn_beta;
   void* bn_acc;
+  int bn_mask_out;
 } buctd_c3_conv;
 int buctd_conv3x3_bf16x6_group(int n, const buctd_c3_conv* convs, void* stream);
 typedef struct {
@@ -162,6 +167,7 @@
 } buctd_bn_acc_in;
 int buctd_bn_apply_acc(const float* z, const buctd_bn_acc_in* st, const float* gamma, const float* beta,
                        const float* residual, int relu, float* y, long rows, int C, void* stream);
+#define BUCTD_BN_RELU_DY_MASKED 2
 int buctd_bn_bwd_acc(const float* dy, const float* y, const float* z, const float* mean, const float* invstd,
                      const float* gamma, const float* beta, int relu, long rows, int C, float* dz, float* dres,
                      float* dgamma, float* dbeta, int accumulate, void* acc, int acc_ready, void* stream);
@@ -319,6 +325,7 @@
 int buctd_basic_branches_fwd_train(int nb, int n, const buctd_basic_block* blocks, void* stream);
 int buctd_basic_branches_bwd(int nb, int n, const buctd_basic_block* blocks, const buctd_basic_block_grads* grads, void* stream,
                              void* side_stream);
+int buctd_basic_row_dy_masked(int nb, int n, const buctd_basic_block* blocks, const buctd_basic_block_grads* grads, int* out);
 
 int buctd_stream_fork(void* from, void* to);
 
```

Measured after the change: 519.5 images/s (median of 6 runs). Within noise of the previous version (+0.7%).
